# gyatskov/radix-sort

Hardware: AMD Instinct MI355X
Metric: Mkeys/s + scatter-pass HBM GB/s (% of peak), 2^28 uint32 keys (higher is better)
Workload: dtype u32; 1 GPU; 2^28 uint32 Random, 4-bit digits, 8 passes; keys_per_gpu=268435456, total_keys=268435456, parallelism=single GPU, verified=bit-exact vs RadixSortCPU (reference), all 268435456 keys

## Files before the change

radix-sort_amd/csrc/rsx_capi.hip:

```cpp
#include "radixsort_hip.h"
#ifdef RSX_EXPERIMENTS
#include "radixsort_hip_experiments.h"
#endif
#include "rsx_kernels.hpp"
#include "rsx_segmented.hpp"
#include "rsx_topk.hpp"
#include "rsx_select.hpp"
#include "rsx_unique.hpp"
#include "rsx_reduce.hpp"
#include "rsx_scan_by_key.hpp"

#include <hip/hip_runtime.h>

#include <algorithm>
#include <cstdio>
#include <cstdlib>
#include <cstring>
#include <limits>
#include <new>
#include <map>
#include <string>
#include <vector>

namespace {

thread_local std::string g_last_error;

int fail(int status, const char* what, hipError_t err = hipSuccess)
{
    g_last_error = what;
    if (err != hipSuccess) {
        g_last_error += ": ";
        g_last_error += hipGetErrorString(err);
    }
    std::fprintf(stderr, "[radixsort_hip] %s\n", g_last_error.c_str());
    return status;
}

#define RSX_TRY(expr, status)                                     \
    do {                                                          \
        const hipError_t rsx_err_ = (expr);                       \
        if (rsx_err_ != hipSuccess) {                             \
            return fail((status), #expr, rsx_err_);               \
        }                                                         \
    } while (0)

#ifndef RSX_TILE_THREADS
#define RSX_TILE_THREADS 256
#endif
#ifndef RSX_KPT
#define RSX_KPT 16
#endif
constexpr int kTileThreads = RSX_TILE_THREADS;
constexpr int kKeysPerThread = RSX_KPT;
constexpr int kTileKeys = kTileThreads * kKeysPerThread;
constexpr int kSmallKeysPerThread = 4;
#define RSX_PRODUCT_SHAPE (RSX_TILE_THREADS == 256 && RSX_KPT == 16)

enum Phase : int { PH_HISTO = 0, PH_SCAN = 1, PH_PASTE = 2, PH_REORDER = 3, PH_TOTAL = 4, PH_COUNT = 5 };

struct EventPair {
    int phase;
    hipEvent_t start, stop;
};

void stat_reset(rsx_phase_stat& s)
{
    s.min_ms = std::numeric_limits<double>::infinity();
    s.max_ms = -std::numeric_limits<double>::infinity();
    s.avg_ms = 0.0;
    s.sum_ms = 0.0;
    s.n = 0;
}

void stat_update(rsx_phase_stat& s, double ms)
{
    s.n += 1;
    s.sum_ms += ms;
    s.avg_ms = s.sum_ms / static_cast<double>(s.n);
    s.max_ms = std::max(s.max_ms, ms);
    s.min_ms = std::min(s.min_ms, ms);
}

}

struct GraphEntry {
    const void* in;
    const uint32_t* pin;
    uint64_t n;
    int cur, first, last, flags;
    uint64_t options_epoch;
    hipStream_t stream;
    hipGraphExec_t exec;
    int end_cur;
    const void* end_last_in;
    int end_last_shift;
};

struct rsx_engine {
    int device = 0;
    int key_bytes = 4;
    bool is_signed = false;
    int key_kind = RSX_KEY_UNSIGNED;
    bool descending = false;
    int codec_first = 0, codec_last = 0;
    bool has_payload = false;
    uint64_t capacity = 0;
    uint64_t n = 0;

    void* keys[2] = {nullptr, nullptr};
    uint32_t* perm[2] = {nullptr, nullptr};
    int cur = 0;
    void* result_keys = nullptr;
    uint32_t* result_perm = nullptr;

    uint32_t* table = nullptr;
    uint32_t* globsum = nullptr;
    uint32_t* globsum2 = nullptr;
    uint32_t* globsum_live = nullptr;
    int paste_scan = 1;
    int fused_scan = 1;
    unsigned long long* gsums = nullptr;
    uint32_t* scan_timeout = nullptr;
    uint32_t* scan_timeout_host = nullptr;
    uint32_t fused_scan_resident = 0;
    uint32_t fused_scan_limit = 0;
    bool table_valid = false;
    bool globsum_valid = false;
    uint32_t scan_epoch = 0;
    uint32_t* temp = nullptr;
    uint32_t* counts_next = nullptr;
#ifdef RSX_EXPERIMENTS
    uint32_t* counts_next2 = nullptr;
    uint32_t* scan_ready = nullptr;
    int inline_scan = 0;
    uint32_t inline_scan_max_groups = 64;
    uint32_t inline_scan_limit = 0;
#endif
#ifdef RSX_STAMPS
    unsigned long long* stamps = nullptr;
    int stamp_pass = -1;
#endif
    uint32_t* ref_table = nullptr;
    uint32_t* ref_globsum = nullptr;
    const void* counted_keys = nullptr;
    uint64_t counted_n = 0;
    int counted_shift = 0, counted_bits = 0;
    const void* last_in = nullptr;
    int last_shift = 0;
    int ref_diag = 0;
    uint64_t splitters[rsx::kMaxSplitters] = {};
    uint32_t nsplit = 0;
    bool result_external = false;
    void* final_keys_out = nullptr;
    uint32_t* final_perm_out = nullptr;
    unsigned long long* range_dev = nullptr;
    unsigned long long* range_host = nullptr;
    uint32_t* starts_dev = nullptr;
    uint32_t* starts_host = nullptr;
    uint64_t table_cap = 0;
#ifdef RSX_EXPERIMENTS
    struct BigBuf {
        void* base = nullptr;
        size_t size = 0;
        std::vector<hipMemGenericAllocationHandle_t> chunks;
    };
    std::vector<BigBuf> big;
    int alloc_mode = 0;
    size_t alloc_chunk = 0;
#endif
    rsx::MsdPlan* msd_plan = nullptr;
    rsx::MsdPlan* msd_plan_host = nullptr;
    uint32_t* msd_starts = nullptr;
    hipEvent_t msd_event = nullptr;
    hipEvent_t msd_scatter_event = nullptr;
    bool msd_scattered = false;
    hipEvent_t marks[RSX_MAX_MARKS] = {};
    std::map<int, hipEvent_t> order_events;
    const void* msd_keys = nullptr;
    uint64_t msd_n = 0;
    int msd_bits = 0, msd_world = 0;
    bool msd_planned = false;

    rsx::SegHeader* seg_hdr = nullptr;
    uint32_t* seg_temp = nullptr;
    uint32_t* seg_status_host = nullptr;
    uint32_t* seg_status = nullptr;
    uint64_t* seg_bsum = nullptr;
    uint32_t* seg_list = nullptr;
    rsx::SegLarge* seg_large = nullptr;
    uint32_t* seg_tstart = nullptr;
    uint32_t* seg_table = nullptr;
    uint32_t* seg_gsum = nullptr;
    uint32_t* seg_gsum2 = nullptr;
    uint64_t seg_bsum_cap = 0, seg_list_cap = 0, seg_large_cap = 0, seg_tstart_cap = 0, seg_table_cap = 0, seg_gsum_cap = 0, seg_gsum2_cap = 0;
    rsx::TopkState* topk_state = nullptr;
    uint32_t* topk_start = nullptr;
    uint32_t* topk_cont = nullptr;
    uint64_t topk_state_cap = 0, topk_start_cap = 0, topk_cont_cap = 0;
    uint32_t* uniq_iota = nullptr;
    uint64_t uniq_iota_cap = 0;
    uint64_t* red_part = nullptr;
    uint64_t red_part_cap = 0;

    hipStream_t stream = nullptr;
    bool own_stream = false;

    struct Pipeline {
        bool ready = false;
        void* in[2] = {nullptr, nullptr};
        void* out[2] = {nullptr, nullptr};
        uint32_t* pin[2] = {nullptr, nullptr};
        uint32_t* pout[2] = {nullptr, nullptr};
        hipStream_t s_in = nullptr, s_out = nullptr;
        hipEvent_t in_ready[2] = {nullptr, nullptr}, sorted[2] = {nullptr, nullptr}, out_done[2] = {nullptr, nullptr};
        uint64_t submitted = 0;
    } pipe;

    int profile = 0;
    int xcd_remap = 1;
    uint64_t options_epoch = 0;
    int64_t xcd_phase = -1;
    int lookahead = 1;
    int small_scan = 1;
    uint64_t radix8_min_keys = 1u << 19;
    int radix_bits = 4;
#ifdef RSX_EXPERIMENTS
    int reorder8_version = 1;
    int r8_stay = -1;
    int lds_atomics_ordered = -1;
    uint32_t* tickets8 = nullptr;
#endif
    long r8_extra_lds = -1;
    long reorder_extra_lds = -1;
    int reorder_wide = -1;
    int r8_wide = -1;
    int num_cus = 0;
    int r8_packed = 1;
    bool radix8_ready = false;
    uint32_t* counts8 = nullptr;
    uint32_t* table8 = nullptr;
    uint32_t* gsum8 = nullptr;
    uint32_t* csum8 = nullptr;
    uint32_t* cbase8 = nullptr;
    int self_scan = 1;
    uint32_t self_scan_max = 1024;
    uint32_t* cnt3[3] = {nullptr, nullptr, nullptr};
    uint64_t small_tile_max_keys = 1u << 19;
    int tile_sort = 1;
    int first_pass = 0;
    int last_pass = 0;

    int use_graph = 0;
    std::vector<GraphEntry> graphs;
    std::vector<EventPair> pending;
    std::vector<hipEvent_t> pool;
    rsx_phase_stat stats[PH_COUNT];

    uint32_t passes() const { return static_cast<uint32_t>(key_bytes * 8 / RSX_RADIX_BITS); }
    bool codec() const { return key_kind == RSX_KEY_FLOAT || descending; }
    uint64_t ntiles(uint64_t count) const { return (count + kTileKeys - 1) / kTileKeys; }
};

namespace {

struct Bracket {
    rsx_engine* e;
    int phase;
    hipEvent_t start = nullptr, stop = nullptr;
    bool on = false;
    Bracket(rsx_engine* eng, int ph) : e(eng), phase(ph)
    {
        if (e->profile == 0 || (e->profile == 2 && ph != PH_REORDER && ph != PH_TOTAL)) return;
        auto take = [&]() -> hipEvent_t {
            if (!e->pool.empty()) {
                hipEvent_t ev = e->pool.back();
                e->pool.pop_back();
                return ev;
            }
            hipEvent_t ev = nullptr;
            if (hipEventCreate(&ev) != hipSuccess) return nullptr;
            return ev;
        };
        start = take();
        stop = take();
        on = start && stop;
        if (on) (void)hipEventRecord(start, e->stream);
    }
    ~Bracket()
    {
        if (!on) return;
        (void)hipEventRecord(stop, e->stream);
        e->pending.push_back({phase, start, stop});
    }
};

int drain_events(rsx_engine* e)
{
    RSX_TRY(hipStreamSynchronize(e->stream), RSX_CALCULATION_FAILED);
    for (const EventPair& p : e->pending) {
        float ms = 0.f;
        if (hipEventElapsedTime(&ms, p.start, p.stop) == hipSuccess) {
            stat_update(e->stats[p.phase], static_cast<double>(ms));
        }
        e->pool.push_back(p.start);
        e->pool.push_back(p.stop);
    }
    e->pending.clear();
    return RSX_OK;
}

template <typename Key>
Key flip_mask(const rsx_engine* e)
{
    return (e->is_signed && !e->codec()) ? static_cast<Key>(Key{1} << (sizeof(Key) * 8 - 1)) : Key{0};
}

template <typename Key>
void order_consts(const rsx_engine* e, Key* a, Key* m)
{
    constexpr Key sign = static_cast<Key>(Key{1} << (sizeof(Key) * 8 - 1));
    if (e->key_kind == RSX_KEY_FLOAT) {
        *m = static_cast<Key>(~sign);
        *a = e->descending ? static_cast<Key>(~sign) : sign;
    } else {
        *m = Key{0};
        const Key flip = e->is_signed ? sign : Key{0};
        *a = e->descending ? static_cast<Key>(~flip) : flip;
    }
}

template <typename Key>
Key codec_decode_host(Key y, Key a, Key m)
{
    const Key z = y ^ a;
    const Key fill = (z >> (sizeof(Key) * 8 - 1)) ? static_cast<Key>(~Key{0}) : Key{0};
    return z ^ (fill & m);
}

constexpr int kEncode = 1, kDecode = 2;

template <typename Key>
rsx::KeyCodec<Key> key_codec(const rsx_engine* e, int cx)
{
    Key a = 0, m = 0;
    order_consts<Key>(e, &a, &m);
    rsx::KeyCodec<Key> c{};
    if (cx & kEncode) {
        c.ea = a;
        c.em = m;
    }
    if (cx & kDecode) {
        c.da = a;
        c.dm = m;
    }
    return c;
}

int pass_codec(const rsx_engine* e, int pass, int width, int first, int last)
{
    if (!e->codec()) return 0;
    return (pass == first ? kEncode : 0) | (pass + width == last ? kDecode : 0);
}
int pass_codec(const rsx_engine* e, int pass, int width)
{
    return pass_codec(e, pass, width, e->codec_first, e->codec_last);
}

int refuse_codec(const char* what)
{
    return fail(RSX_CALCULATION_FAILED, (std::string(what) + ": not available for float keys or descending order (the sharded sort and the partition passes take integer keys in ascending order)").c_str());
}

struct Grid {
    uint32_t ntiles, tiles_per_xcd, blocks;
    int remap;
};

Grid grid_for(const rsx_engine* e, uint64_t count, uint32_t tile_keys = kTileKeys)
{
    Grid g;
    g.ntiles = static_cast<uint32_t>((count + tile_keys - 1) / tile_keys);
    g.tiles_per_xcd = (g.ntiles + rsx::kNumXcd - 1) / rsx::kNumXcd;
    g.blocks = e->xcd_remap ? g.tiles_per_xcd * rsx::kNumXcd : g.ntiles;
    const uint64_t want = e->xcd_phase < 0 ? g.tiles_per_xcd / rsx::kNumXcd : static_cast<uint64_t>(e->xcd_phase);
    const uint32_t phase = (e->xcd_remap && (rsx::kNumXcd - 1) * want < g.tiles_per_xcd) ? static_cast<uint32_t>(want) : 0u;
    g.remap = (e->xcd_remap ? 1 : 0) | static_cast<int>(phase << 8);
    return g;
}

template <typename Key>
rsx::SplitSet<Key> split_set(const rsx_engine* e, uint32_t nsplit)
{
    rsx::SplitSet<Key> set{};
    for (uint32_t k = 0; k < nsplit && k < static_cast<uint32_t>(rsx::kMaxSplitters); ++k) set.s[k] = static_cast<Key>(e->splitters[k]);
    set.n = nsplit;
    return set;
}

template <typename Key, bool RANGED = false>
int launch_histogram(rsx_engine* e, const void* in, uint64_t count, int shift, uint32_t mask, Key lo = Key{0}, Key mul = Key{0}, uint32_t nsplit = 0,
                     int cx = 0)
{
    if (count == 0) return RSX_OK;
    e->counted_keys = nullptr;
    e->table_valid = true;
    e->globsum_valid = false;
    const Grid g = grid_for(e, count);
    Bracket b(e, PH_HISTO);
    if (!RANGED && (cx & kEncode)) {
        hipLaunchKernelGGL((rsx::histogram_kernel<Key, kTileThreads, kKeysPerThread, false, true>), dim3(g.blocks), dim3(kTileThreads), 0, e->stream,
                           static_cast<const Key*>(in), e->table, count, g.ntiles, g.tiles_per_xcd, g.remap, shift,
                           flip_mask<Key>(e), mask, lo, mul, split_set<Key>(e, nsplit), nullptr, nullptr, nullptr, key_codec<Key>(e, kEncode));
    } else {
        hipLaunchKernelGGL((rsx::histogram_kernel<Key, kTileThreads, kKeysPerThread, RANGED>), dim3(g.blocks), dim3(kTileThreads), 0, e->stream,
                           static_cast<const Key*>(in), e->table, count, g.ntiles, g.tiles_per_xcd, g.remap, shift,
                           flip_mask<Key>(e), mask, lo, mul, split_set<Key>(e, nsplit));
    }
    RSX_TRY(hipGetLastError(), RSX_CALCULATION_FAILED);
    return RSX_OK;
}

int launch_scan(rsx_engine* e, uint64_t count, bool from_counts = false, bool scan_level2 = true)
{
    if (count == 0) return RSX_OK;
    e->counted_keys = nullptr;
    const uint32_t ntiles = static_cast<uint32_t>(e->ntiles(count));
    const uint32_t ngroups = (ntiles + rsx::kScanTiles - 1) / rsx::kScanTiles;
    e->globsum_live = e->globsum;
    e->table_valid = true;
    e->globsum_valid = true;
    {
        Bracket b(e, PH_SCAN);
        if (from_counts) {
            hipLaunchKernelGGL((rsx::scan_blocks_kernel<true, true>), dim3(ngroups), dim3(rsx::kScanTiles), 0, e->stream, e->table, e->globsum,
                               ntiles, ngroups, e->counts_next);
        } else {
            hipLaunchKernelGGL((rsx::scan_blocks_kernel<false, false>), dim3(ngroups), dim3(rsx::kScanTiles), 0, e->stream, e->table, e->globsum,
                               ntiles, ngroups, static_cast<uint32_t*>(nullptr));
        }
    }
    RSX_TRY(hipGetLastError(), RSX_CALCULATION_FAILED);
    if (scan_level2) {
        Bracket b(e, PH_SCAN);
        hipLaunchKernelGGL(rsx::scan_globsum_kernel, dim3(1), dim3(rsx::kGlobsumThreads), 0, e->stream, e->globsum, e->temp,
                           static_cast<uint32_t>(RSX_RADIX) * ngroups);
    }
    RSX_TRY(hipGetLastError(), RSX_CALCULATION_FAILED);
    return RSX_OK;
}

int launch_paste_scan(rsx_engine* e, uint64_t count)
{
    if (count == 0) return RSX_OK;
    const uint32_t ntiles = static_cast<uint32_t>(e->ntiles(count));
    const uint32_t ngroups = (ntiles + rsx::kScanTiles - 1) / rsx::kScanTiles;
    e->globsum_live = e->globsum2;
    e->globsum_valid = true;
    Bracket b(e, PH_PASTE);
    hipLaunchKernelGGL(rsx::paste_scan_kernel, dim3(ngroups), dim3(rsx::kScanTiles), 0, e->stream, e->table, e->globsum, e->globsum2, e->temp,
                       ntiles, ngroups);
    RSX_TRY(hipGetLastError(), RSX_CALCULATION_FAILED);
    return RSX_OK;
}

bool launch_scan_fused(rsx_engine* e, uint64_t count, bool from_counts, int* rc)
{
    const uint32_t ntiles = static_cast<uint32_t>(e->ntiles(count));
    const uint32_t ngroups = (ntiles + rsx::kScanTiles - 1) / rsx::kScanTiles;
    if (!e->fused_scan || e->use_graph || count == 0 || ngroups > e->fused_scan_limit) return false;
    e->counted_keys = nullptr;
    e->globsum_live = e->globsum2;
    e->table_valid = true;
    e->globsum_valid = true;
    if (++e->scan_epoch == 0) e->scan_epoch = 1;
    {
        Bracket b(e, PH_SCAN);
        if (from_counts) {
            hipLaunchKernelGGL((rsx::scan_fused_kernel<true, true>), dim3(ngroups), dim3(rsx::kScanTiles), 0, e->stream, e->table, e->gsums, e->globsum2, e->temp,
                               ntiles, ngroups, e->counts_next, e->scan_epoch, e->scan_timeout);
        } else {
            hipLaunchKernelGGL((rsx::scan_fused_kernel<false, false>), dim3(ngroups), dim3(rsx::kScanTiles), 0, e->stream, e->table, e->gsums, e->globsum2, e->temp,
                               ntiles, ngroups, e->counts_next, e->scan_epoch, e->scan_timeout);
        }
    }
    *rc = hipGetLastError() == hipSuccess ? RSX_OK : fail(RSX_CALCULATION_FAILED, "scan_fused_kernel launch");
    return true;
}

bool launch_scan_small(rsx_engine* e, uint64_t count, bool from_counts, int* rc)
{
    const uint32_t ntiles = static_cast<uint32_t>(e->ntiles(count));
    if (!e->small_scan || count == 0 || ntiles > static_cast<uint32_t>(rsx::kSmallScanMaxTiles)) return false;
    e->counted_keys = nullptr;
    e->table_valid = true;
    e->globsum_valid = false;
    {
        Bracket b(e, PH_SCAN);
        if (from_counts) {
            hipLaunchKernelGGL((rsx::scan_small_kernel<true, true>), dim3(1), dim3(rsx::kSmallScanThreads), 0, e->stream, e->table, e->counts_next, e->temp, ntiles);
        } else {
            hipLaunchKernelGGL((rsx::scan_small_kernel<false, false>), dim3(1), dim3(rsx::kSmallScanThreads), 0, e->stream, e->table, e->counts_next, e->temp, ntiles);
        }
    }
    *rc = hipGetLastError() == hipSuccess ? RSX_OK : fail(RSX_CALCULATION_FAILED, "scan_small_kernel launch");
    return true;
}

int launch_paste(rsx_engine* e, uint64_t count)
{
    if (count == 0) return RSX_OK;
    const uint32_t ntiles = static_cast<uint32_t>(e->ntiles(count));
    const uint32_t ngroups = (ntiles + rsx::kScanTiles - 1) / rsx::kScanTiles;
    Bracket b(e, PH_PASTE);
    hipLaunchKernelGGL(rsx::paste_kernel, dim3(ngroups), dim3(rsx::kScanTiles), 0, e->stream, e->table, e->globsum, ntiles, ngroups);
    RSX_TRY(hipGetLastError(), RSX_CALCULATION_FAILED);
    return RSX_OK;
}

template <typename Key, bool PAYLOAD, bool LOOKAHEAD, bool RANGED = false, int KPT = kKeysPerThread, int THREADS = kTileThreads>
int launch_reorder_t(rsx_engine* e, const void* in, void* out, const uint32_t* pin, uint32_t* pout, uint64_t count, int shift,
                     uint32_t mask, int next_shift, Key lo = Key{0}, Key mul = Key{0}, uint32_t nsplit = 0,
                     rsx::SelfScanArgs self = rsx::SelfScanArgs{nullptr, nullptr, nullptr}, uint32_t* next_counts = nullptr, int cx = 0)
{
    using L = rsx::ReorderLayout<Key, THREADS, KPT>;
    const Grid g = grid_for(e, count, THREADS * KPT);
    e->last_in = in;
    e->last_shift = shift;
    Bracket b(e, PH_REORDER);
    const size_t lds = L::BYTES + (KPT != kKeysPerThread ? 0u : e->reorder_extra_lds >= 0 ? static_cast<size_t>(e->reorder_extra_lds) : (PAYLOAD && sizeof(Key) == 4 && !RANGED) ? (16u << 10) : 0u);
    if constexpr (!RANGED) {
        if (cx) {
            hipLaunchKernelGGL((rsx::reorder_kernel<Key, THREADS, KPT, PAYLOAD, LOOKAHEAD, false, false, true>), dim3(g.blocks), dim3(THREADS), lds,
                               e->stream, static_cast<const Key*>(in), static_cast<Key*>(out), pin, pout, e->table, count,
                               g.ntiles, g.tiles_per_xcd, g.remap, shift, flip_mask<Key>(e), mask,
                               next_counts ? next_counts : e->counts_next, next_shift, static_cast<const uint32_t*>(nullptr),
                               lo, mul, split_set<Key>(e, nsplit), self, rsx::InlineScanArgs{}, key_codec<Key>(e, cx));
            RSX_TRY(hipGetLastError(), RSX_CALCULATION_FAILED);
            return RSX_OK;
        }
    }
    hipLaunchKernelGGL((rsx::reorder_kernel<Key, THREADS, KPT, PAYLOAD, LOOKAHEAD, RANGED>), dim3(g.blocks), dim3(THREADS),
                       lds,
                       e->stream, static_cast<const Key*>(in), static_cast<Key*>(out), pin, pout, e->table, count,
                       g.ntiles, g.tiles_per_xcd, g.remap, shift, flip_mask<Key>(e), mask,
                       next_counts ? next_counts : e->counts_next, next_shift,
#ifdef RSX_STAMPS
                       (shift == e->stamp_pass * RSX_RADIX_BITS) ? reinterpret_cast<const uint32_t*>(e->stamps) : static_cast<const uint32_t*>(nullptr),
#else
                       static_cast<const uint32_t*>(nullptr),
#endif
                       lo, mul, split_set<Key>(e, nsplit), self);
    RSX_TRY(hipGetLastError(), RSX_CALCULATION_FAILED);
    return RSX_OK;
}

template <typename Key>
int launch_reorder(rsx_engine* e, const void* in, void* out, const uint32_t* pin, uint32_t* pout, uint64_t count, int shift,
                   uint32_t mask, int next_shift = -1, int cx = 0)
{
    const rsx::SelfScanArgs none{nullptr, nullptr, nullptr};
    if (count == 0) return RSX_OK;
    const bool payload = pin && pout;
#if RSX_PRODUCT_SHAPE
    if constexpr (sizeof(Key) == 8) {
        if (payload && (e->reorder_wide >= 0 ? e->reorder_wide != 0 : true)) {
            return next_shift >= 0 ? launch_reorder_t<Key, true, true, false, 8, 512>(e, in, out, pin, pout, count, shift, mask, next_shift, Key{0}, Key{0}, 0, none, nullptr, cx)
                                   : launch_reorder_t<Key, true, false, false, 8, 512>(e, in, out, pin, pout, count, shift, mask, 0, Key{0}, Key{0}, 0, none, nullptr, cx);
        }
    }
#endif
    if (next_shift >= 0) {
        return payload ? launch_reorder_t<Key, true, true>(e, in, out, pin, pout, count, shift, mask, next_shift, Key{0}, Key{0}, 0, none, nullptr, cx)
                       : launch_reorder_t<Key, false, true>(e, in, out, nullptr, nullptr, count, shift, mask, next_shift, Key{0}, Key{0}, 0, none, nullptr, cx);
    }
    return payload ? launch_reorder_t<Key, true, false>(e, in, out, pin, pout, count, shift, mask, 0, Key{0}, Key{0}, 0, none, nullptr, cx)
                   : launch_reorder_t<Key, false, false>(e, in, out, nullptr, nullptr, count, shift, mask, 0, Key{0}, Key{0}, 0, none, nullptr, cx);
}

int no_static_lds(const void* fn, const char* name)
{
    hipFuncAttributes attr;
    RSX_TRY(hipFuncGetAttributes(&attr, fn), RSX_KERNEL_CREATION_FAILED);
    if (attr.sharedSizeBytes != 0) return fail(RSX_KERNEL_CREATION_FAILED, (std::string(name) + ": static LDS in front of the dynamic array (the kernels address LDS from 0)").c_str());
    return RSX_OK;
}

int lds_base_probe(rsx_engine* e)
{
    uint32_t at = 1;
    RSX_TRY(hipMemsetAsync(e->temp + 4, 0xFF, 4, e->stream), RSX_KERNEL_CREATION_FAILED);
    hipLaunchKernelGGL(rsx::lds_base_probe_kernel, dim3(1), dim3(64), 256, e->stream, e->temp + 4);
    RSX_TRY(hipGetLastError(), RSX_KERNEL_CREATION_FAILED);
    RSX_TRY(hipMemcpyAsync(&at, e->temp + 4, 4, hipMemcpyDeviceToHost, e->stream), RSX_KERNEL_CREATION_FAILED);
    RSX_TRY(hipStreamSynchronize(e->stream), RSX_KERNEL_CREATION_FAILED);
    if (at != 0) return fail(RSX_KERNEL_CREATION_FAILED, "a kernel's dynamic LDS does not start at address 0 on this device");
    return RSX_OK;
}

template <typename Key, bool PAYLOAD, bool LOOKAHEAD, bool RANGED = false, int KPT = kKeysPerThread, int THREADS = kTileThreads, bool CODEC = false>
int allow_lds()
{
    using L = rsx::ReorderLayout<Key, THREADS, KPT>;
    const void* fn = reinterpret_cast<const void*>(&rsx::reorder_kernel<Key, THREADS, KPT, PAYLOAD, LOOKAHEAD, RANGED, false, CODEC>);
    RSX_TRY(hipFuncSetAttribute(fn, hipFuncAttributeMaxDynamicSharedMemorySize, static_cast<int>(L::BYTES) + (64 << 10)), RSX_INITIALIZATION_FAILED);
    return no_static_lds(fn, "reorder_kernel");
}

template <typename Key>
int run_pass(rsx_engine* e, const void* in, void* out, const uint32_t* pin, uint32_t* pout, uint64_t count, int shift, uint32_t mask, int cx = 0)
{
    int rc;
    if ((rc = launch_histogram<Key>(e, in, count, shift, mask, Key{0}, Key{0}, 0, cx)) != RSX_OK) return rc;
    if ((rc = launch_scan(e, count)) != RSX_OK) return rc;
    if ((rc = launch_paste(e, count)) != RSX_OK) return rc;
    return launch_reorder<Key>(e, in, out, pin, pout, count, shift, mask, -1, cx);
}

template <typename Key>
int run_ranged_pass(rsx_engine* e, const void* in, void* out, const uint32_t* pin, uint32_t* pout, uint64_t count, uint64_t lo, int shift,
                    uint64_t mul)
{
    const Key klo = static_cast<Key>(lo), kmul = static_cast<Key>(mul);
    int rc;
    if ((rc = launch_histogram<Key, true>(e, in, count, shift, RSX_RADIX - 1, klo, kmul)) != RSX_OK) return rc;
    if ((rc = launch_scan(e, count)) != RSX_OK) return rc;
    if ((rc = launch_paste(e, count)) != RSX_OK) return rc;
    if (pin && pout) return launch_reorder_t<Key, true, false, true>(e, in, out, pin, pout, count, shift, RSX_RADIX - 1, 0, klo, kmul);
    return launch_reorder_t<Key, false, false, true>(e, in, out, nullptr, nullptr, count, shift, RSX_RADIX - 1, 0, klo, kmul);
}

constexpr int kRangeBlocks = 2048;

template <typename Key>
int key_range(rsx_engine* e, const void* d_keys, uint64_t n, uint64_t* lo, uint64_t* hi)
{
    const uint32_t blocks = static_cast<uint32_t>(std::min<uint64_t>(kRangeBlocks, (n + 4095) / 4096));
    hipLaunchKernelGGL(rsx::key_range_kernel<Key>, dim3(blocks), dim3(rsx::kRangeThreads), 0, e->stream, static_cast<const Key*>(d_keys), n,
                       flip_mask<Key>(e), e->range_dev);
    RSX_TRY(hipGetLastError(), RSX_CALCULATION_FAILED);
    RSX_TRY(hipMemcpyAsync(e->range_host, e->range_dev, static_cast<size_t>(blocks) * 16, hipMemcpyDeviceToHost, e->stream), RSX_CALCULATION_FAILED);
    RSX_TRY(hipStreamSynchronize(e->stream), RSX_CALCULATION_FAILED);
    unsigned long long l = ~0ull, h = 0ull;
    for (uint32_t b = 0; b < blocks; ++b) {
        l = std::min(l, e->range_host[2 * b]);
        h = std::max(h, e->range_host[2 * b + 1]);
    }
    *lo = l;
    *hi = h;
    return RSX_OK;
}

template <typename Key, bool PAYLOAD>
int launch_tile_sort_t(rsx_engine* e, const void* in, void* out, void* before_last, const uint32_t* pin, uint32_t* pout, uint32_t* pbefore_last, uint64_t count)
{
    using L = rsx::TileSortLayout<Key, kTileThreads, kKeysPerThread>;
    Bracket b(e, PH_REORDER);
    if (e->codec()) {
        hipLaunchKernelGGL((rsx::tile_sort_kernel<Key, kTileThreads, kKeysPerThread, PAYLOAD, true>), dim3(1), dim3(kTileThreads), L::BYTES, e->stream,
                           static_cast<const Key*>(in), static_cast<Key*>(out), static_cast<Key*>(before_last), pin, pout, pbefore_last,
                           static_cast<uint32_t>(count), e->first_pass, e->last_pass, flip_mask<Key>(e), e->table, e->globsum, e->temp,
                           key_codec<Key>(e, pass_codec(e, e->first_pass, e->last_pass - e->first_pass)));
    } else {
        hipLaunchKernelGGL((rsx::tile_sort_kernel<Key, kTileThreads, kKeysPerThread, PAYLOAD>), dim3(1), dim3(kTileThreads), L::BYTES, e->stream,
                           static_cast<const Key*>(in), static_cast<Key*>(out), static_cast<Key*>(before_last), pin, pout, pbefore_last,
                           static_cast<uint32_t>(count), e->first_pass, e->last_pass, flip_mask<Key>(e), e->table, e->globsum, e->temp);
    }
    RSX_TRY(hipGetLastError(), RSX_CALCULATION_FAILED);
    return RSX_OK;
}

template <typename Key>
int sort_tile_enqueue(rsx_engine* e, const void* ext_keys, const uint32_t* ext_perm, uint64_t count)
{
    const int npasses = e->last_pass - e->first_pass;
    const void* in = ext_keys ? ext_keys : e->keys[e->cur];
    const uint32_t* pin = e->has_payload ? (ext_keys ? ext_perm : e->perm[e->cur]) : nullptr;
    const int first_dst = ext_keys ? e->cur : (e->cur ^ 1);
    const int final_buf = first_dst ^ ((npasses - 1) & 1);
    void* out = e->final_keys_out ? e->final_keys_out : e->keys[final_buf];
    uint32_t* pout = e->has_payload ? (e->final_keys_out ? e->final_perm_out : e->perm[final_buf]) : nullptr;
    void* before_last = npasses > 1 ? e->keys[final_buf ^ 1] : nullptr;
    uint32_t* pbefore_last = (npasses > 1 && e->has_payload) ? e->perm[final_buf ^ 1] : nullptr;
    Bracket whole(e, PH_TOTAL);
    e->counted_keys = nullptr;
    e->globsum_live = e->globsum;
    const int rc = e->has_payload ? launch_tile_sort_t<Key, true>(e, in, out, before_last, pin, pout, pbefore_last, count)
                                  : launch_tile_sort_t<Key, false>(e, in, out, before_last, nullptr, nullptr, nullptr, count);
    if (rc != RSX_OK) return rc;
    e->last_in = npasses > 1 ? before_last : in;
    e->last_shift = (e->last_pass - 1) * RSX_RADIX_BITS;
    e->table_valid = true;
    e->globsum_valid = true;
    e->result_external = e->final_keys_out != nullptr;
    if (e->final_keys_out) {
        e->result_keys = e->final_keys_out;
        e->result_perm = e->has_payload ? e->final_perm_out : nullptr;
    } else {
        e->cur = final_buf;
        e->result_keys = e->keys[e->cur];
        e->result_perm = e->has_payload ? e->perm[e->cur] : nullptr;
    }
    return RSX_OK;
}

template <typename Key, int KPT = kKeysPerThread>
int sort_selfscan_enqueue(rsx_engine* e, const void* ext_keys, const uint32_t* ext_perm, uint64_t count)
{
    const Grid g = grid_for(e, count, kTileThreads * KPT);
    const void* in = ext_keys ? ext_keys : e->keys[e->cur];
    const uint32_t* pin = e->has_payload ? (ext_keys ? ext_perm : e->perm[e->cur]) : nullptr;
    int dst = ext_keys ? e->cur : (e->cur ^ 1);
    Bracket whole(e, PH_TOTAL);
    e->counted_keys = nullptr;
    {
        Bracket b(e, PH_HISTO);
        if (pass_codec(e, e->first_pass, 1) & kEncode) {
            hipLaunchKernelGGL((rsx::histogram_kernel<Key, kTileThreads, KPT, false, true>), dim3(g.blocks), dim3(kTileThreads), 0, e->stream,
                               static_cast<const Key*>(in), e->table, count, g.ntiles, g.tiles_per_xcd, g.remap, e->first_pass * RSX_RADIX_BITS,
                               flip_mask<Key>(e), static_cast<uint32_t>(RSX_RADIX - 1), Key{0}, Key{0}, split_set<Key>(e, 0), e->cnt3[0], e->cnt3[1], e->cnt3[2],
                               key_codec<Key>(e, kEncode));
        } else {
            hipLaunchKernelGGL((rsx::histogram_kernel<Key, kTileThreads, KPT, false>), dim3(g.blocks), dim3(kTileThreads), 0, e->stream,
                               static_cast<const Key*>(in), e->table, count, g.ntiles, g.tiles_per_xcd, g.remap, e->first_pass * RSX_RADIX_BITS,
                               flip_mask<Key>(e), static_cast<uint32_t>(RSX_RADIX - 1), Key{0}, Key{0}, split_set<Key>(e, 0), e->cnt3[0], e->cnt3[1], e->cnt3[2]);
        }
        RSX_TRY(hipGetLastError(), RSX_CALCULATION_FAILED);
    }
    int i = 0;
    for (int pass = e->first_pass; pass < e->last_pass; ++pass, ++i) {
        const bool last = pass + 1 == e->last_pass;
        const bool to_caller = e->final_keys_out && last;
        void* out = to_caller ? e->final_keys_out : e->keys[dst];
        uint32_t* pout = e->has_payload ? (to_caller ? e->final_perm_out : e->perm[dst]) : nullptr;
        const int shift = pass * RSX_RADIX_BITS;
        const rsx::SelfScanArgs self{e->cnt3[i % 3], e->cnt3[(i + 2) % 3], (last && KPT == kKeysPerThread) ? e->table : nullptr};
        uint32_t* next = e->cnt3[(i + 1) % 3];
        const int cx = pass_codec(e, pass, 1);
        int rc;
        if (e->has_payload) {
            rc = last ? launch_reorder_t<Key, true, false, false, KPT>(e, in, out, pin, pout, count, shift, RSX_RADIX - 1, 0, Key{0}, Key{0}, 0, self, next, cx)
                      : launch_reorder_t<Key, true, true, false, KPT>(e, in, out, pin, pout, count, shift, RSX_RADIX - 1, shift + RSX_RADIX_BITS, Key{0}, Key{0}, 0, self, next, cx);
        } else {
            rc = last ? launch_reorder_t<Key, false, false, false, KPT>(e, in, out, nullptr, nullptr, count, shift, RSX_RADIX - 1, 0, Key{0}, Key{0}, 0, self, next, cx)
                      : launch_reorder_t<Key, false, true, false, KPT>(e, in, out, nullptr, nullptr, count, shift, RSX_RADIX - 1, shift + RSX_RADIX_BITS, Key{0}, Key{0}, 0, self, next, cx);
        }
        if (rc != RSX_OK) return rc;
        in = out;
        pin = pout;
        dst ^= 1;
    }
    e->table_valid = (KPT == kKeysPerThread);
    e->globsum_valid = false;
    if (in == e->keys[0] || in == e->keys[1]) e->cur = (in == e->keys[0]) ? 0 : 1;
    e->result_external = e->final_keys_out != nullptr;
    if (e->final_keys_out) {
        e->result_keys = e->final_keys_out;
        e->result_perm = e->has_payload ? e->final_perm_out : nullptr;
    } else {
        e->result_keys = e->keys[e->cur];
        e->result_perm = e->has_payload ? e->perm[e->cur] : nullptr;
    }
    return RSX_OK;
}

#if RSX_TILE_THREADS == 256
size_t r8_extra_lds_for(const rsx_engine* e, bool elem64, bool separate_payload)
{
    if (e->r8_extra_lds >= 0) return static_cast<size_t>(e->r8_extra_lds);
    if (!elem64) return separate_payload ? 0 : (4u << 10);
    if (separate_payload) return 16u << 10;
    return 8u << 10;
}

bool r8_wide_for(const rsx_engine* e, bool key64, bool has_payload)
{
    if (e->r8_wide >= 0) return e->r8_wide != 0;
    return key64 && !has_payload;
}

template <typename K, int THREADS, int KPT, bool PAYLOAD, bool PACKED32 = false, bool CODEC = false>
int allow_lds8(int extra)
{
    using L = rsx::Reorder8Layout<K, THREADS, KPT, PAYLOAD>;
    const void* fn = reinterpret_cast<const void*>(&rsx::reorder8_kernel<K, THREADS, KPT, PAYLOAD, PACKED32, CODEC>);
    RSX_TRY(hipFuncSetAttribute(fn, hipFuncAttributeMaxDynamicSharedMemorySize, static_cast<int>(L::BYTES) + extra), RSX_INITIALIZATION_FAILED);
    return no_static_lds(fn, "reorder8_kernel");
}

#ifdef RSX_EXPERIMENTS
template <typename Key> int ensure_radix8_experiments(rsx_engine* e, int extra);
template <typename Key> bool launch_reorder8_experiment(rsx_engine* e, const void* in, void* out, const uint32_t* pin, uint32_t* pout, uint64_t count, const Grid& g,
                                                        uint32_t chunk_groups, int shift, int byte_pass, bool first_of_chain, int* rc);
#endif

template <typename Key>
int ensure_radix8(rsx_engine* e)
{
    if (e->radix8_ready) return RSX_OK;
    const int extra = e->r8_extra_lds >= 0 ? static_cast<int>(e->r8_extra_lds) : (16 << 10);
    const size_t rows = static_cast<size_t>(e->ntiles(e->capacity)) * rsx::kRadix8 * 4;
    const size_t groups = ((e->ntiles(e->capacity) + rsx::kScan8Tiles - 1) / rsx::kScan8Tiles) * rsx::kRadix8 * 4;
    if (!e->counts8) RSX_TRY(hipMalloc(reinterpret_cast<void**>(&e->counts8), rows), RSX_INITIALIZATION_FAILED);
    if (!e->table8) RSX_TRY(hipMalloc(reinterpret_cast<void**>(&e->table8), rows), RSX_INITIALIZATION_FAILED);
    if (!e->gsum8) RSX_TRY(hipMalloc(reinterpret_cast<void**>(&e->gsum8), groups), RSX_INITIALIZATION_FAILED);
    if (!e->csum8) RSX_TRY(hipMalloc(reinterpret_cast<void**>(&e->csum8), rsx::kScan8MaxChunks * rsx::kRadix8 * 4), RSX_INITIALIZATION_FAILED);
    if (!e->cbase8) RSX_TRY(hipMalloc(reinterpret_cast<void**>(&e->cbase8), rsx::kScan8MaxChunks * rsx::kRadix8 * 4), RSX_INITIALIZATION_FAILED);
    int rc = allow_lds8<Key, kTileThreads, kKeysPerThread, false>(extra);
    if (rc == RSX_OK) rc = allow_lds8<Key, kTileThreads, kKeysPerThread, true>(extra);
    if (rc == RSX_OK) rc = allow_lds8<Key, 512, 8, false>(extra);
    if (rc == RSX_OK) rc = allow_lds8<Key, 512, 8, true>(extra);
    if constexpr (sizeof(Key) == 4) {
        if (rc == RSX_OK) rc = allow_lds8<uint64_t, kTileThreads, kKeysPerThread, false, true>(extra);
        if (rc == RSX_OK) rc = allow_lds8<uint64_t, 512, 8, false, true>(extra);
    }
    if (e->codec()) {
        if (rc == RSX_OK) rc = allow_lds8<Key, kTileThreads, kKeysPerThread, false, false, true>(extra);
        if (rc == RSX_OK) rc = allow_lds8<Key, kTileThreads, kKeysPerThread, true, false, true>(extra);
        if (rc == RSX_OK) rc = allow_lds8<Key, 512, 8, false, false, true>(extra);
        if (rc == RSX_OK) rc = allow_lds8<Key, 512, 8, true, false, true>(extra);
        if constexpr (sizeof(Key) == 4) {
            if (rc == RSX_OK) rc = allow_lds8<uint64_t, kTileThreads, kKeysPerThread, false, true, true>(extra);
            if (rc == RSX_OK) rc = allow_lds8<uint64_t, 512, 8, false, true, true>(extra);
        }
    }
#ifdef RSX_EXPERIMENTS
    if (rc == RSX_OK) rc = ensure_radix8_experiments<Key>(e, extra);
#endif
    if (rc != RSX_OK) return rc;
    e->radix8_ready = true;
    return RSX_OK;
}

template <typename K, int THREADS, int KPT, bool PAYLOAD, bool PACKED32 = false>
void launch_reorder8_v(rsx_engine* e, const dim3& grid, size_t lds, const void* in, void* out, const uint32_t* pin, uint32_t* pout, uint64_t count,
                       const Grid& g, uint32_t chunk_groups, int shift, K flip, int cx)
{
    using CK = typename std::conditional<PACKED32, uint32_t, K>::type;
    if (cx) {
        hipLaunchKernelGGL((rsx::reorder8_kernel<K, THREADS, KPT, PAYLOAD, PACKED32, true>), grid, dim3(THREADS), lds, e->stream,
                           static_cast<const K*>(in), static_cast<K*>(out), pin, pout, e->table8, e->gsum8, e->cbase8, chunk_groups,
                           count, g.ntiles, g.tiles_per_xcd, g.remap, shift, flip, key_codec<CK>(e, cx));
    } else {
        hipLaunchKernelGGL((rsx::reorder8_kernel<K, THREADS, KPT, PAYLOAD, PACKED32>), grid, dim3(THREADS), lds, e->stream,
                           static_cast<const K*>(in), static_cast<K*>(out), pin, pout, e->table8, e->gsum8, e->cbase8, chunk_groups,
                           count, g.ntiles, g.tiles_per_xcd, g.remap, shift, flip);
    }
}

template <typename Key>
int launch_reorder8(rsx_engine* e, const void* in, void* out, const uint32_t* pin, uint32_t* pout, uint64_t count, const Grid& g, uint32_t chunk_groups, int shift,
                    int cx = 0)
{
    const Key flip = flip_mask<Key>(e);
    e->last_in = nullptr;
    const bool packed = sizeof(Key) == 4 && e->has_payload && e->r8_packed;
    const bool wide = r8_wide_for(e, sizeof(Key) == 8, e->has_payload);
    const size_t wide_extra = e->r8_extra_lds >= 0 ? static_cast<size_t>(e->r8_extra_lds) : 0;
    const dim3 grid(g.blocks);
    constexpr size_t lds_packed = rsx::Reorder8Layout<uint64_t, kTileThreads, kKeysPerThread>::BYTES, lds_packed_wide = rsx::Reorder8Layout<uint64_t, 512, 8, false>::BYTES;
    constexpr size_t lds_pay = rsx::Reorder8Layout<Key, kTileThreads, kKeysPerThread, true>::BYTES, lds_pay_wide = rsx::Reorder8Layout<Key, 512, 8, true>::BYTES;
    constexpr size_t lds_keys = rsx::Reorder8Layout<Key, kTileThreads, kKeysPerThread>::BYTES, lds_keys_wide = rsx::Reorder8Layout<Key, 512, 8, false>::BYTES;
    if (packed) {
        if (wide) {
            launch_reorder8_v<uint64_t, 512, 8, false, true>(e, grid, lds_packed_wide + wide_extra, in, out, pin, pout, count, g, chunk_groups, shift,
                                                             static_cast<uint64_t>(flip), cx);
        } else {
            launch_reorder8_v<uint64_t, kTileThreads, kKeysPerThread, false, true>(e, grid, lds_packed + r8_extra_lds_for(e, true, false), in, out, pin, pout, count, g,
                                                                                   chunk_groups, shift, static_cast<uint64_t>(flip), cx);
        }
    } else if (e->has_payload) {
        if (wide) {
            launch_reorder8_v<Key, 512, 8, true>(e, grid, lds_pay_wide + wide_extra, in, out, pin, pout, count, g, chunk_groups, shift, flip, cx);
        } else {
            launch_reorder8_v<Key, kTileThreads, kKeysPerThread, true>(e, grid, lds_pay + r8_extra_lds_for(e, sizeof(Key) == 8, true), in, out, pin, pout, count, g,
                                                                      chunk_groups, shift, flip, cx);
        }
    } else {
        if (wide) {
            launch_reorder8_v<Key, 512, 8, false>(e, grid, lds_keys_wide + wide_extra, in, out, nullptr, nullptr, count, g, chunk_groups, shift, flip, cx);
        } else {
            launch_reorder8_v<Key, kTileThreads, kKeysPerThread, false>(e, grid, lds_keys + r8_extra_lds_for(e, sizeof(Key) == 8, false), in, out, nullptr, nullptr,
                                                                       count, g, chunk_groups, shift, flip, cx);
        }
    }
    RSX_TRY(hipGetLastError(), RSX_CALCULATION_FAILED);
    return RSX_OK;
}

struct Scan8Shape {
    uint32_t ngroups, chunk_groups, nchunks;
};
Scan8Shape scan8_shape(uint32_t ntiles)
{
    Scan8Shape s;
    s.ngroups = (ntiles + rsx::kScan8Tiles - 1) / rsx::kScan8Tiles;
    s.chunk_groups = std::max<uint32_t>(64u, (s.ngroups + rsx::kScan8MaxChunks - 1) / rsx::kScan8MaxChunks);
    s.nchunks = (s.ngroups + s.chunk_groups - 1) / s.chunk_groups;
    return s;
}

template <typename Key>
int launch_count8(rsx_engine* e, const void* in, uint64_t count, const Grid& g, const Scan8Shape& s, int shift, int cx = 0)
{
    e->msd_keys = nullptr;
    {
        Bracket b(e, PH_HISTO);
        if (cx & kEncode) {
            hipLaunchKernelGGL((rsx::histogram8_kernel<Key, kTileThreads, kKeysPerThread, true>), dim3(g.blocks), dim3(kTileThreads), 0, e->stream,
                               static_cast<const Key*>(in), e->counts8, count, g.ntiles, g.tiles_per_xcd, g.remap, shift, flip_mask<Key>(e), key_codec<Key>(e, kEncode));
        } else {
            hipLaunchKernelGGL((rsx::histogram8_kernel<Key, kTileThreads, kKeysPerThread>), dim3(g.blocks), dim3(kTileThreads), 0, e->stream,
                               static_cast<const Key*>(in), e->counts8, count, g.ntiles, g.tiles_per_xcd, g.remap, shift, flip_mask<Key>(e));
        }
    }
    {
        Bracket b(e, PH_SCAN);
        hipLaunchKernelGGL(rsx::scan8_blocks_kernel, dim3(s.ngroups), dim3(rsx::kRadix8), 0, e->stream, e->counts8, e->table8, e->gsum8, g.ntiles);
    }
    {
        Bracket b(e, PH_SCAN);
        if (s.nchunks == 1) {
            hipLaunchKernelGGL(rsx::scan8_chunks_kernel<true>, dim3(1), dim3(rsx::kRadix8), 0, e->stream, e->gsum8, e->csum8, s.ngroups, s.chunk_groups, e->cbase8, e->temp);
        } else {
            hipLaunchKernelGGL(rsx::scan8_chunks_kernel<false>, dim3(s.nchunks), dim3(rsx::kRadix8), 0, e->stream, e->gsum8, e->csum8, s.ngroups, s.chunk_groups, e->cbase8, e->temp);
            hipLaunchKernelGGL(rsx::scan8_top_kernel, dim3(1), dim3(rsx::kRadix8), 0, e->stream, e->csum8, e->cbase8, e->temp, s.nchunks);
        }
    }
    RSX_TRY(hipGetLastError(), RSX_CALCULATION_FAILED);
    return RSX_OK;
}

template <typename Key>
int sort8_chain_enqueue(rsx_engine* e, const void* ext_keys, const uint32_t* ext_perm, uint64_t count)
{
    const Grid g = grid_for(e, count);
    const Scan8Shape s = scan8_shape(g.ntiles);
    if (!e->radix8_ready) return fail(RSX_INITIALIZATION_FAILED, "sort8_chain_enqueue: the 8-bit tables were not allocated (ensure_radix8)");
    const void* in = ext_keys ? ext_keys : e->keys[e->cur];
    const uint32_t* pin = e->has_payload ? (ext_keys ? ext_perm : e->perm[e->cur]) : nullptr;
    int dst = ext_keys ? e->cur : (e->cur ^ 1);
    Bracket whole(e, PH_TOTAL);
    e->counted_keys = nullptr;
    for (int pass = e->first_pass; pass < e->last_pass; pass += 2) {
        const bool to_caller = e->final_keys_out && pass + 2 == e->last_pass;
        void* out = to_caller ? e->final_keys_out : e->keys[dst];
        uint32_t* pout = e->has_payload ? (to_caller ? e->final_perm_out : e->perm[dst]) : nullptr;
        const int shift = pass * RSX_RADIX_BITS;
        const int cx = pass_codec(e, pass, 2);
        int rc = launch_count8<Key>(e, in, count, g, s, shift, cx);
        if (rc != RSX_OK) return rc;
        {
            Bracket b(e, PH_REORDER);
#ifdef RSX_EXPERIMENTS
            if (e->codec() || !launch_reorder8_experiment<Key>(e, in, out, pin, pout, count, g, s.chunk_groups, shift, pass / 2, pass == e->first_pass, &rc))
#endif
                rc = launch_reorder8<Key>(e, in, out, pin, pout, count, g, s.chunk_groups, shift, cx);
        }
        if (rc != RSX_OK) return rc;
        in = out;
        pin = pout;
        dst ^= 1;
    }
    e->table_valid = false;
    e->globsum_valid = false;
    if (in == e->keys[0] || in == e->keys[1]) e->cur = (in == e->keys[0]) ? 0 : 1;
    e->result_external = e->final_keys_out != nullptr;
    if (e->final_keys_out) {
        e->result_keys = e->final_keys_out;
        e->result_perm = e->has_payload ? e->final_perm_out : nullptr;
    } else {
        e->result_keys = e->keys[e->cur];
        e->result_perm = e->has_payload ? e->perm[e->cur] : nullptr;
    }
    return RSX_OK;
}

#endif

#ifdef RSX_EXPERIMENTS
template <typename Key> int sort_inline_enqueue(rsx_engine* e, const void* ext_keys, const uint32_t* ext_perm, uint64_t count);
bool inline_scan_takes(const rsx_engine* e, uint64_t count);
#endif

template <typename Key>
int sort_chain_passes(rsx_engine* e, const void* ext_keys, const uint32_t* ext_perm, uint64_t count);

template <typename Key>
int sort_chain_enqueue(rsx_engine* e, const void* ext_keys, const uint32_t* ext_perm, uint64_t count)
{
    e->codec_first = e->first_pass;
    e->codec_last = e->last_pass;
    return sort_chain_passes<Key>(e, ext_keys, ext_perm, count);
}

template <typename Key>
int sort_chain_passes(rsx_engine* e, const void* ext_keys, const uint32_t* ext_perm, uint64_t count)
{
#if RSX_TILE_THREADS == 256
    if (e->radix_bits == 8 && count > e->radix8_min_keys && e->first_pass < e->last_pass && (e->first_pass & 1) == 0 && (e->last_pass & 1) == 0) {
        return sort8_chain_enqueue<Key>(e, ext_keys, ext_perm, count);
    }
    if (e->radix_bits == 8 && count > e->radix8_min_keys && (e->first_pass & 1) == 0 && (e->last_pass & 1) == 1 && e->last_pass - e->first_pass >= 3) {
        const int first = e->first_pass, last = e->last_pass;
        void* const keys_out = e->final_keys_out;
        uint32_t* const perm_out = e->final_perm_out;
        e->last_pass = last - 1;
        e->final_keys_out = nullptr;
        e->final_perm_out = nullptr;
        int rc = sort8_chain_enqueue<Key>(e, ext_keys, ext_perm, count);
        e->last_pass = last;
        e->final_keys_out = keys_out;
        e->final_perm_out = perm_out;
        if (rc != RSX_OK) return rc;
        e->first_pass = last - 1;
        rc = sort_chain_passes<Key>(e, nullptr, nullptr, count);
        e->first_pass = first;
        return rc;
    }
#endif
#if RSX_PRODUCT_SHAPE
    if (e->tile_sort && e->profile != 1 && count > 0 && count <= static_cast<uint64_t>(kTileKeys) && e->first_pass < e->last_pass) {
        return sort_tile_enqueue<Key>(e, ext_keys, ext_perm, count);
    }
#endif
    if (e->self_scan && e->lookahead && count > static_cast<uint64_t>(kTileKeys) && e->ntiles(count) <= e->self_scan_max && e->first_pass < e->last_pass) {
        if (count <= e->small_tile_max_keys) return sort_selfscan_enqueue<Key, kSmallKeysPerThread>(e, ext_keys, ext_perm, count);
        return sort_selfscan_enqueue<Key>(e, ext_keys, ext_perm, count);
    }
#if defined(RSX_EXPERIMENTS) && RSX_PRODUCT_SHAPE
    if (!e->codec() && inline_scan_takes(e, count)) return sort_inline_enqueue<Key>(e, ext_keys, ext_perm, count);
#endif
    const void* in = ext_keys ? ext_keys : e->keys[e->cur];
    const uint32_t* pin = e->has_payload ? (ext_keys ? ext_perm : e->perm[e->cur]) : nullptr;
    int dst = ext_keys ? e->cur : (e->cur ^ 1);
    Bracket whole(e, PH_TOTAL);
    if (e->lookahead && count > 0) {
        RSX_TRY(hipMemsetAsync(e->counts_next, 0, static_cast<size_t>(e->ntiles(count)) * RSX_RADIX * 4, e->stream), RSX_CALCULATION_FAILED);
    }
    for (int pass = e->first_pass; pass < e->last_pass; ++pass) {
        const bool to_caller = e->final_keys_out && pass + 1 == e->last_pass;
        void* out = to_caller ? e->final_keys_out : e->keys[dst];
        uint32_t* pout = e->has_payload ? (to_caller ? e->final_perm_out : e->perm[dst]) : nullptr;
        const int shift = pass * RSX_RADIX_BITS;
        const int cx = pass_codec(e, pass, 1);
        int rc;
        if (!e->lookahead) {
            rc = run_pass<Key>(e, in, out, pin, pout, count, shift, RSX_RADIX - 1, cx);
        } else {
            const bool first = pass == e->first_pass;
            rc = first ? launch_histogram<Key>(e, in, count, shift, RSX_RADIX - 1, Key{0}, Key{0}, 0, cx) : RSX_OK;
            bool pasted = false;
            if (rc == RSX_OK) pasted = launch_scan_small(e, count, !first, &rc);
            if (rc == RSX_OK && !pasted) pasted = launch_scan_fused(e, count, !first, &rc);
            const bool merged = e->paste_scan != 0;
            if (rc == RSX_OK && !pasted) rc = launch_scan(e, count, !first, !merged);
            const bool last = pass + 1 == e->last_pass;
            if (rc == RSX_OK && !pasted) rc = merged ? launch_paste_scan(e, count) : launch_paste(e, count);
            const int next_shift = last ? -1 : shift + RSX_RADIX_BITS;
            if (rc == RSX_OK) rc = launch_reorder<Key>(e, in, out, pin, pout, count, shift, RSX_RADIX - 1, next_shift, cx);
        }
        if (rc != RSX_OK) return rc;
        in = out;
        pin = pout;
        dst ^= 1;
    }
    if (in == e->keys[0] || in == e->keys[1]) {
        e->cur = (in == e->keys[0]) ? 0 : 1;
    }
    e->result_external = e->final_keys_out != nullptr;
    if (e->final_keys_out) {
        e->result_keys = e->final_keys_out;
        e->result_perm = e->has_payload ? e->final_perm_out : nullptr;
    } else {
        e->result_keys = e->keys[e->cur];
        e->result_perm = e->has_payload ? e->perm[e->cur] : nullptr;
    }
    return RSX_OK;
}

constexpr uint64_t kGraphMaxKeys = 1ull << 22;

template <typename Key>
int sort_chain(rsx_engine* e, const void* ext_keys, const uint32_t* ext_perm, uint64_t count)
{
#if RSX_TILE_THREADS == 256
    if (e->radix_bits == 8 && count > e->radix8_min_keys) {
        const int rc8 = ensure_radix8<Key>(e);
        if (rc8 != RSX_OK) return rc8;
    }
#endif
    const bool graphable = e->use_graph && e->profile == 0 && count > 0 && count <= kGraphMaxKeys && e->stream != nullptr && !e->final_keys_out;
    if (!graphable) return sort_chain_enqueue<Key>(e, ext_keys, ext_perm, count);
    GraphEntry key{};
    key.in = ext_keys;
    key.pin = ext_perm;
    key.n = count;
    key.cur = e->cur;
    key.first = e->first_pass;
    key.last = e->last_pass;
    key.flags = (e->lookahead ? 1 : 0) | (e->xcd_remap ? 2 : 0) | (e->small_scan ? 16 : 0);
    key.options_epoch = e->options_epoch;
    key.stream = e->stream;
    for (const GraphEntry& g : e->graphs) {
        if (g.in == key.in && g.pin == key.pin && g.n == key.n && g.cur == key.cur && g.first == key.first && g.last == key.last &&
            g.flags == key.flags && g.options_epoch == key.options_epoch && g.stream == key.stream) {
            RSX_TRY(hipGraphLaunch(g.exec, e->stream), RSX_CALCULATION_FAILED);
            e->cur = g.end_cur;
            e->last_in = g.end_last_in;
            e->last_shift = g.end_last_shift;
            e->result_external = false;
            e->result_keys = e->keys[e->cur];
            e->result_perm = e->has_payload ? e->perm[e->cur] : nullptr;
            return RSX_OK;
        }
    }
    hipGraph_t graph = nullptr;
    if (hipStreamBeginCapture(e->stream, hipStreamCaptureModeThreadLocal) != hipSuccess) {
        (void)hipGetLastError();
        e->use_graph = 0;
        return sort_chain_enqueue<Key>(e, ext_keys, ext_perm, count);
    }
    const int rc = sort_chain_enqueue<Key>(e, ext_keys, ext_perm, count);
    const hipError_t end = hipStreamEndCapture(e->stream, &graph);
    if (rc != RSX_OK || end != hipSuccess || !graph) {
        if (graph) (void)hipGraphDestroy(graph);
        return rc != RSX_OK ? rc : fail(RSX_CALCULATION_FAILED, "hipStreamEndCapture", end);
    }
    hipGraphExec_t exec = nullptr;
    const hipError_t inst = hipGraphInstantiate(&exec, graph, nullptr, nullptr, 0);
    (void)hipGraphDestroy(graph);
    if (inst != hipSuccess) return fail(RSX_CALCULATION_FAILED, "hipGraphInstantiate", inst);
    key.exec = exec;
    key.end_cur = e->cur;
    key.end_last_in = e->last_in;
    key.end_last_shift = e->last_shift;
    if (e->graphs.size() >= 8) {
        (void)hipGraphExecDestroy(e->graphs.front().exec);
        e->graphs.erase(e->graphs.begin());
    }
    e->graphs.push_back(key);
    RSX_TRY(hipGraphLaunch(exec, e->stream), RSX_CALCULATION_FAILED);
    return RSX_OK;
}

template <typename Key>
int sort_chain_keys_only(rsx_engine* e, const void* ext_keys, uint64_t count)
{
    const bool saved = e->has_payload;
    e->has_payload = false;
    const int rc = sort_chain<Key>(e, ext_keys, nullptr, count);
    e->has_payload = saved;
    return rc;
}

int check_scan_timeout(rsx_engine* e, int status)
{
    if (e->seg_status_host) {
        volatile uint32_t* bad = e->seg_status_host;
        const uint32_t v = *bad;
        if (v != 0) {
            *bad = 0;
            return fail(status, ("rsx_segmented_sort / rsx_segmented_topk / rsx_segmented_select: segment " + std::to_string(v - 1) + " has off[s+1] < off[s] or off[s+1] > n; it was neither read nor "
                                 "written (the first such segment of the call; reported once; the engine remains usable)").c_str());
        }
    }
    if (!e->scan_timeout_host) return RSX_OK;
    volatile uint32_t* flag = e->scan_timeout_host;
    if (*flag != 0) {
        *flag = 0;
        return fail(status, "the fused table scan timed out waiting for a group sum: the result of that sort is undefined (reported once; the engine remains usable)");
    }
    return RSX_OK;
}
bool aligned16(const void* p)
{
    return (reinterpret_cast<uintptr_t>(p) & 15u) == 0;
}

bool overlaps(const void* a, uint64_t abytes, const void* b, uint64_t bbytes)
{
    const uintptr_t a0 = reinterpret_cast<uintptr_t>(a), b0 = reinterpret_cast<uintptr_t>(b);
    return a && b && abytes && bbytes && a0 < b0 + bbytes && b0 < a0 + abytes;
}

int alias_of(const void* p, uint64_t bytes, void* const bufs[2], uint64_t buf_bytes, int* which)
{
    for (int i = 0; i < 2; ++i) {
        if (!bufs[i] || !overlaps(p, bytes, bufs[i], buf_bytes)) continue;
        if (p == bufs[i]) {
            *which = i;
            return 1;
        }
        return -1;
    }
    return 0;
}

int bind_device(const rsx_engine* e, int status)
{
    RSX_TRY(hipSetDevice(e->device), status);
    return RSX_OK;
}

#ifdef RSX_EXPERIMENTS
hipError_t big_alloc(rsx_engine* e, void** out, size_t bytes);
bool big_free(rsx_engine* e, void* p);
#else
hipError_t big_alloc(rsx_engine*, void** out, size_t bytes)
{
    *out = nullptr;
    return hipMalloc(out, bytes);
}

bool big_free(rsx_engine*, void* p)
{
    return !p || hipFree(p) == hipSuccess;
}
#endif

#ifdef RSX_EXPERIMENTS
#include "capi_experiments.inc"
#endif

struct EnvKnob {
    const char* name;
    const char* meaning;
    void (*apply)(rsx_engine* e, const char* value);
};
constexpr long kb_or_policy(const char* v, int max_kb)
{
    return std::atoi(v) < 0 ? -1L : static_cast<long>(std::min(max_kb, std::atoi(v))) * 1024;
}
const EnvKnob kEnvKnobs[] = {
    {"RSX_XCD_REMAP", "0: workgroup b takes tile b (default 1: XCD-contiguous tile ranges)", [](rsx_engine* e, const char* v) { e->xcd_remap = std::atoi(v) != 0; }},
    {"RSX_XCD_PHASE", "tiles by which consecutive XCDs enter their range staggered (-1: an eighth of a range)", [](rsx_engine* e, const char* v) { e->xcd_phase = std::atoll(v); }},
    {"RSX_LOOKAHEAD", "0: every pass runs histogram -> scan -> paste -> reorder (default 1: RSX_OPT_LOOKAHEAD)", [](rsx_engine* e, const char* v) { e->lookahead = std::atoi(v) != 0; }},
    {"RSX_GRAPH", "1: small sorts replay a captured hipGraph (RSX_OPT_GRAPH, default 0)", [](rsx_engine* e, const char* v) { e->use_graph = std::atoi(v) != 0; }},
    {"RSX_SMALL_SCAN", "0: no one-workgroup table scan (RSX_OPT_SMALL_SCAN)", [](rsx_engine* e, const char* v) { e->small_scan = std::atoi(v) != 0; }},
    {"RSX_TILE_SORT", "0: no one-launch sort of inputs up to one tile (RSX_OPT_TILE_SORT)", [](rsx_engine* e, const char* v) { e->tile_sort = std::atoi(v) != 0; }},
    {"RSX_SELF_SCAN", "0: small tables get scan launches (RSX_OPT_SELF_SCAN)", [](rsx_engine* e, const char* v) { e->self_scan = std::atoi(v) != 0; }},
    {"RSX_SELF_SCAN_MAX", "largest table, in tiles, of the self-scan chain (RSX_OPT_SELF_SCAN_MAX_TILES)",
     [](rsx_engine* e, const char* v) { e->self_scan_max = std::min<uint32_t>(static_cast<uint32_t>(std::atoi(v)), rsx::kSelfScanMaxTiles); }},
    {"RSX_SMALL_TILE_MAX_KEYS", "self-scan sorts up to this many keys use 1024-key tiles (RSX_OPT_SMALL_TILE_MAX_KEYS)",
     [](rsx_engine* e, const char* v) { e->small_tile_max_keys = std::min<uint64_t>(std::strtoull(v, nullptr, 10), static_cast<uint64_t>(rsx::kSelfScanMaxTiles) * kTileThreads * kSmallKeysPerThread); }},
    {"RSX_PASTE_SCAN", "0: scan #2 gets a launch of its own in the two-launch table scan", [](rsx_engine* e, const char* v) { e->paste_scan = std::atoi(v) != 0; }},
    {"RSX_FUSED_SCAN", "0: never the one-launch table scan (RSX_OPT_FUSED_SCAN)", [](rsx_engine* e, const char* v) { e->fused_scan = std::atoi(v) != 0; }},
    {"RSX_RADIX_BITS", "8: byte-wide passes in the sort chain (RSX_OPT_RADIX_BITS)", [](rsx_engine* e, const char* v) { e->radix_bits = std::atoi(v) == 8 ? 8 : 4; }},
    {"RSX_RADIX8_MIN_KEYS", "8-bit passes only above this many keys (default 2^19)", [](rsx_engine* e, const char* v) { e->radix8_min_keys = std::max<uint64_t>(std::strtoull(v, nullptr, 10), kTileKeys); }},
    {"RSX_REORDER_EXTRA_LDS_KB", "unused dynamic LDS per 4-bit scatter workgroup = fewer per CU (-1: per-variant policy)", [](rsx_engine* e, const char* v) { e->reorder_extra_lds = kb_or_policy(v, 64); }},
    {"RSX_REORDER_WIDE", "4-bit scatter of 64-bit keys + payload on 512 x 8 (0 / 1, -1: policy = on)", [](rsx_engine* e, const char* v) { e->reorder_wide = std::max(-1, std::min(1, std::atoi(v))); }},
    {"RSX_R8_EXTRA_LDS_KB", "the same for the 8-bit scatter (-1: per-variant policy)", [](rsx_engine* e, const char* v) { e->r8_extra_lds = kb_or_policy(v, 96); }},
    {"RSX_R8_PACKED", "0: uint32 key and payload travel apart through the 8-bit scatter (default 1: one 64-bit element)", [](rsx_engine* e, const char* v) { e->r8_packed = std::atoi(v) != 0; }},
    {"RSX_R8_WIDE", "8-bit scatter on 512 x 8 (0 / 1, -1: policy = 64-bit keys without payload)", [](rsx_engine* e, const char* v) { e->r8_wide = std::max(-1, std::min(1, std::atoi(v))); }},
#ifdef RSX_EXPERIMENTS
    {"RSX_ALLOC_MODE", "experiments: key buffers as VMM chunks mapped in creation (1) or shuffled (2) order", [](rsx_engine* e, const char* v) { e->alloc_mode = std::max(0, std::min(2, std::atoi(v))); }},
    {"RSX_ALLOC_CHUNK_MB", "experiments: chunk size of RSX_ALLOC_MODE", [](rsx_engine* e, const char* v) { e->alloc_chunk = static_cast<size_t>(std::max(0, std::atoi(v))) << 20; }},
#endif
};

void apply_environment(rsx_engine* e)
{
    for (const EnvKnob& k : kEnvKnobs) {
        if (const char* v = std::getenv(k.name)) k.apply(e, v);
    }
}

}

#define RSX_BY_KEY(e, call32, call64) ((e)->key_bytes == 4 ? (call32) : (call64))

extern "C" {

const char* rsx_last_error(void)
{
    return g_last_error.c_str();
}

const char* rsx_version(void)
{
    return "radixsort_hip 0.1 (gfx950; tile 256x16; 4-bit LSD)";
}

int rsx_device_count(int* count)
{
    if (!count) return fail(RSX_INITIALIZATION_FAILED, "rsx_device_count: null argument");
    *count = 0;
    int c = 0;
    const hipError_t err = hipGetDeviceCount(&c);
    if (err != hipSuccess) {
        return fail(RSX_INITIALIZATION_FAILED, "hipGetDeviceCount", err);
    }
    *count = c;
    return RSX_OK;
}

int rsx_device_name(int device, char* buf, size_t buflen)
{
    if (!buf || buflen == 0) return fail(RSX_INITIALIZATION_FAILED, "rsx_device_name: null buffer");
    hipDeviceProp_t prop;
    RSX_TRY(hipGetDeviceProperties(&prop, device), RSX_INITIALIZATION_FAILED);
    std::snprintf(buf, buflen, "%s (%s, %d CUs)", prop.name, prop.gcnArchName, prop.multiProcessorCount);
    return RSX_OK;
}

int rsx_create(rsx_engine** out, int device, int key_bytes, int key_kind, int has_payload, uint64_t capacity)
{
    if (!out) return fail(RSX_INITIALIZATION_FAILED, "rsx_create: null out pointer");
    *out = nullptr;
    if (key_bytes != 4 && key_bytes != 8) return fail(RSX_INITIALIZATION_FAILED, "rsx_create: key_bytes must be 4 or 8");
    if (key_kind < RSX_KEY_UNSIGNED || key_kind > RSX_KEY_FLOAT)
        return fail(RSX_INITIALIZATION_FAILED, "rsx_create: key_kind must be RSX_KEY_UNSIGNED (0), RSX_KEY_SIGNED (1) or RSX_KEY_FLOAT (2)");
    if (capacity == 0 || capacity > 0xFFFFFFFFull) {
        return fail(RSX_RESIZE_FAILED, "rsx_create: capacity must be in [1, 2^32-1] (32-bit slots)");
    }
    int count = 0;
    if (rsx_device_count(&count) != RSX_OK || count <= 0) {
        return fail(RSX_INITIALIZATION_FAILED, "rsx_create: no HIP device (this library has no CPU fallback)");
    }
    if (device < 0 || device >= count) return fail(RSX_INITIALIZATION_FAILED, "rsx_create: device ordinal out of range");

    rsx_engine* e = new (std::nothrow) rsx_engine();
    if (!e) return fail(RSX_HOST_BUFFERS_FAILED, "rsx_create: out of host memory");
    e->device = device;
    e->key_bytes = key_bytes;
    e->key_kind = key_kind;
    e->is_signed = key_kind == RSX_KEY_SIGNED;
    e->has_payload = has_payload != 0;
    e->capacity = capacity;
    e->n = 0;
    e->last_pass = static_cast<int>(e->passes());
    for (auto& s : e->stats) stat_reset(s);
    apply_environment(e);

    auto bail = [&](int status, const char* what, hipError_t err) {
        rsx_destroy(e);
        return fail(status, what, err);
    };
    hipError_t err;
    if ((err = hipSetDevice(device)) != hipSuccess) return bail(RSX_INITIALIZATION_FAILED, "hipSetDevice", err);
    if ((err = hipStreamCreateWithFlags(&e->stream, hipStreamNonBlocking)) != hipSuccess)
        return bail(RSX_INITIALIZATION_FAILED, "hipStreamCreate", err);
    e->own_stream = true;

    const size_t key_buf = static_cast<size_t>(capacity) * key_bytes;
    for (int i = 0; i < 2; ++i) {
        if ((err = big_alloc(e, &e->keys[i], key_buf)) != hipSuccess) return bail(RSX_INITIALIZATION_FAILED, "allocation of a key buffer", err);
        if (e->has_payload) {
            if ((err = big_alloc(e, reinterpret_cast<void**>(&e->perm[i]), static_cast<size_t>(capacity) * 4)) != hipSuccess)
                return bail(RSX_INITIALIZATION_FAILED, "hipMalloc(permutations)", err);
        }
    }
    e->table_cap = static_cast<uint64_t>(RSX_RADIX) * e->ntiles(capacity);
    if ((e->ntiles(capacity) + rsx::kScanTiles - 1) / rsx::kScanTiles > rsx::kMaxScanGroups) {
        return bail(RSX_RESIZE_FAILED, "rsx_create: capacity exceeds the two-level table scan", hipSuccess);
    }
    const size_t table_alloc = ((e->ntiles(capacity) + rsx::kScanTiles - 1) / rsx::kScanTiles) * rsx::kScanTiles * RSX_RADIX * 4;
    if ((err = hipMalloc(reinterpret_cast<void**>(&e->table), table_alloc)) != hipSuccess)
        return bail(RSX_INITIALIZATION_FAILED, "hipMalloc(histograms)", err);
    if ((err = hipMalloc(reinterpret_cast<void**>(&e->counts_next), table_alloc)) != hipSuccess)
        return bail(RSX_INITIALIZATION_FAILED, "hipMalloc(look-ahead counts)", err);
#ifdef RSX_EXPERIMENTS
    {
        const size_t second = std::min<size_t>(table_alloc, static_cast<size_t>(rsx::kFusedScanMaxGroups) * rsx::kScanTiles * RSX_RADIX * 4);
        if ((err = hipMalloc(reinterpret_cast<void**>(&e->counts_next2), second)) != hipSuccess)
            return bail(RSX_INITIALIZATION_FAILED, "hipMalloc(second look-ahead counts)", err);
        if ((err = hipMemsetAsync(e->counts_next2, 0, second, e->stream)) != hipSuccess)
            return bail(RSX_INITIALIZATION_FAILED, "hipMemsetAsync(second look-ahead counts)", err);
        if ((err = hipMalloc(reinterpret_cast<void**>(&e->scan_ready), rsx::kFusedScanMaxGroups * 4)) != hipSuccess)
            return bail(RSX_INITIALIZATION_FAILED, "hipMalloc(scan ready words)", err);
        if ((err = hipMemsetAsync(e->scan_ready, 0, rsx::kFusedScanMaxGroups * 4, e->stream)) != hipSuccess)
            return bail(RSX_INITIALIZATION_FAILED, "hipMemsetAsync(scan ready words)", err);
    }
#endif
#ifdef RSX_STAMPS
    if ((err = hipMalloc(reinterpret_cast<void**>(&e->stamps), e->ntiles(capacity) * 16 * 8)) != hipSuccess)
        return bail(RSX_INITIALIZATION_FAILED, "hipMalloc(stamps)", err);
    if (const char* env = std::getenv("RSX_STAMP_PASS")) e->stamp_pass = std::atoi(env);
#endif
    if ((err = hipMalloc(reinterpret_cast<void**>(&e->globsum), rsx::kMaxScanBlocks * 4)) != hipSuccess)
        return bail(RSX_INITIALIZATION_FAILED, "hipMalloc(globsum)", err);
    if ((err = hipMalloc(reinterpret_cast<void**>(&e->globsum2), rsx::kMaxScanBlocks * 4)) != hipSuccess)
        return bail(RSX_INITIALIZATION_FAILED, "hipMalloc(globsum2)", err);
    e->globsum_live = e->globsum;
    if ((err = hipMalloc(reinterpret_cast<void**>(&e->temp), 64)) != hipSuccess)
        return bail(RSX_INITIALIZATION_FAILED, "hipMalloc(temp)", err);
    for (int i = 0; i < 3; ++i) {
        if ((err = hipMalloc(reinterpret_cast<void**>(&e->cnt3[i]), rsx::kSelfScanMaxTiles * RSX_RADIX * 4)) != hipSuccess)
            return bail(RSX_INITIALIZATION_FAILED, "hipMalloc(self-scan counts)", err);
    }
    if ((err = hipMalloc(reinterpret_cast<void**>(&e->gsums), rsx::kFusedScanMaxGroups * RSX_RADIX * 8)) != hipSuccess)
        return bail(RSX_INITIALIZATION_FAILED, "hipMalloc(group sums)", err);
    if ((err = hipMemsetAsync(e->gsums, 0, rsx::kFusedScanMaxGroups * RSX_RADIX * 8, e->stream)) != hipSuccess)
        return bail(RSX_INITIALIZATION_FAILED, "hipMemsetAsync(group sums)", err);
    if ((err = hipHostMalloc(reinterpret_cast<void**>(&e->scan_timeout_host), 64, hipHostMallocMapped)) != hipSuccess)
        return bail(RSX_HOST_BUFFERS_FAILED, "hipHostMalloc(scan timeout flag)", err);
    e->scan_timeout_host[0] = 0;
    if ((err = hipHostGetDevicePointer(reinterpret_cast<void**>(&e->scan_timeout), e->scan_timeout_host, 0)) != hipSuccess)
        return bail(RSX_HOST_BUFFERS_FAILED, "hipHostGetDevicePointer(scan timeout flag)", err);
    {
        int per_cu = 0, cus = 0;
        if ((err = hipOccupancyMaxActiveBlocksPerMultiprocessor(&per_cu, reinterpret_cast<const void*>(&rsx::scan_fused_kernel<true, true>), rsx::kScanTiles, 0)) != hipSuccess)
            return bail(RSX_INITIALIZATION_FAILED, "hipOccupancyMaxActiveBlocksPerMultiprocessor(scan_fused_kernel)", err);
        if ((err = hipDeviceGetAttribute(&cus, hipDeviceAttributeMultiprocessorCount, device)) != hipSuccess)
            return bail(RSX_INITIALIZATION_FAILED, "hipDeviceGetAttribute(multiProcessorCount)", err);
        e->num_cus = cus;
        e->fused_scan_resident = static_cast<uint32_t>(std::max(per_cu, 0)) * static_cast<uint32_t>(std::max(cus, 0));
        e->fused_scan_limit = std::min<uint32_t>(e->fused_scan_resident / 2, rsx::kFusedScanMaxGroups);
        if (const char* env = std::getenv("RSX_FUSED_SCAN_MAX_GROUPS"))
            e->fused_scan_limit = std::min<uint32_t>(static_cast<uint32_t>(std::max(0, std::atoi(env))), std::min<uint32_t>(e->fused_scan_resident, rsx::kFusedScanMaxGroups));
    }
    if ((err = hipMalloc(reinterpret_cast<void**>(&e->ref_table), rsx::kRefTable * 4)) != hipSuccess)
        return bail(RSX_INITIALIZATION_FAILED, "hipMalloc(ref table)", err);
    if ((err = hipMalloc(reinterpret_cast<void**>(&e->ref_globsum), rsx::kRefSplit * 4)) != hipSuccess)
        return bail(RSX_INITIALIZATION_FAILED, "hipMalloc(ref globsum)", err);
    if ((err = hipMalloc(reinterpret_cast<void**>(&e->range_dev), kRangeBlocks * 16)) != hipSuccess)
        return bail(RSX_INITIALIZATION_FAILED, "hipMalloc(range)", err);
    if ((err = hipHostMalloc(reinterpret_cast<void**>(&e->range_host), kRangeBlocks * 16, hipHostMallocDefault)) != hipSuccess)
        return bail(RSX_HOST_BUFFERS_FAILED, "hipHostMalloc(range)", err);
    if ((err = hipMalloc(reinterpret_cast<void**>(&e->starts_dev), RSX_RADIX * 4)) != hipSuccess)
        return bail(RSX_INITIALIZATION_FAILED, "hipMalloc(starts)", err);
    if ((err = hipHostMalloc(reinterpret_cast<void**>(&e->starts_host), RSX_RADIX * 4, hipHostMallocDefault)) != hipSuccess)
        return bail(RSX_HOST_BUFFERS_FAILED, "hipHostMalloc(starts)", err);
    if ((err = hipMemsetAsync(e->globsum, 0, rsx::kMaxScanBlocks * 4, e->stream)) != hipSuccess)
        return bail(RSX_INITIALIZATION_FAILED, "hipMemsetAsync(globsum)", err);

    int rc = lds_base_probe(e);
#if RSX_PRODUCT_SHAPE
    if (rc == RSX_OK) {
        auto allow_tile = [](const void* fn, size_t bytes) { return hipFuncSetAttribute(fn, hipFuncAttributeMaxDynamicSharedMemorySize, static_cast<int>(bytes)); };
        using L32 = rsx::TileSortLayout<uint32_t, kTileThreads, kKeysPerThread>;
        using L64 = rsx::TileSortLayout<uint64_t, kTileThreads, kKeysPerThread>;
        if (allow_tile(reinterpret_cast<const void*>(&rsx::tile_sort_kernel<uint32_t, kTileThreads, kKeysPerThread, false>), L32::BYTES) != hipSuccess ||
            allow_tile(reinterpret_cast<const void*>(&rsx::tile_sort_kernel<uint32_t, kTileThreads, kKeysPerThread, true>), L32::BYTES) != hipSuccess ||
            allow_tile(reinterpret_cast<const void*>(&rsx::tile_sort_kernel<uint64_t, kTileThreads, kKeysPerThread, false>), L64::BYTES) != hipSuccess ||
            allow_tile(reinterpret_cast<const void*>(&rsx::tile_sort_kernel<uint64_t, kTileThreads, kKeysPerThread, true>), L64::BYTES) != hipSuccess ||
            allow_tile(reinterpret_cast<const void*>(&rsx::tile_sort_kernel<uint32_t, kTileThreads, kKeysPerThread, false, true>), L32::BYTES) != hipSuccess ||
            allow_tile(reinterpret_cast<const void*>(&rsx::tile_sort_kernel<uint32_t, kTileThreads, kKeysPerThread, true, true>), L32::BYTES) != hipSuccess ||
            allow_tile(reinterpret_cast<const void*>(&rsx::tile_sort_kernel<uint64_t, kTileThreads, kKeysPerThread, false, true>), L64::BYTES) != hipSuccess ||
            allow_tile(reinterpret_cast<const void*>(&rsx::tile_sort_kernel<uint64_t, kTileThreads, kKeysPerThread, true, true>), L64::BYTES) != hipSuccess)
            rc = fail(RSX_INITIALIZATION_FAILED, "hipFuncSetAttribute(tile_sort_kernel)");
    }
#endif
#if RSX_PRODUCT_SHAPE
    if (rc == RSX_OK) rc = allow_lds<uint64_t, true, false, false, 8, 512>();
    if (rc == RSX_OK) rc = allow_lds<uint64_t, true, true, false, 8, 512>();
    if (rc == RSX_OK) rc = allow_lds<uint64_t, true, false, false, 8, 512, true>();
    if (rc == RSX_OK) rc = allow_lds<uint64_t, true, true, false, 8, 512, true>();
#endif
    if (rc == RSX_OK) rc = allow_lds<uint32_t, false, false>();
    if (rc == RSX_OK) rc = allow_lds<uint32_t, true, false>();
    if (rc == RSX_OK) rc = allow_lds<uint64_t, false, false>();
    if (rc == RSX_OK) rc = allow_lds<uint64_t, true, false>();
    if (rc == RSX_OK) rc = allow_lds<uint32_t, false, true>();
    if (rc == RSX_OK) rc = allow_lds<uint32_t, true, true>();
    if (rc == RSX_OK) rc = allow_lds<uint64_t, false, true>();
    if (rc == RSX_OK) rc = allow_lds<uint64_t, true, true>();
    if (rc == RSX_OK) rc = allow_lds<uint32_t, false, false, true>();
    if (rc == RSX_OK) rc = allow_lds<uint32_t, true, false, true>();
    if (rc == RSX_OK) rc = allow_lds<uint64_t, false, false, true>();
    if (rc == RSX_OK) rc = allow_lds<uint64_t, true, false, true>();
    if (rc == RSX_OK) rc = allow_lds<uint32_t, false, false, false, kKeysPerThread, kTileThreads, true>();
    if (rc == RSX_OK) rc = allow_lds<uint32_t, true, false, false, kKeysPerThread, kTileThreads, true>();
    if (rc == RSX_OK) rc = allow_lds<uint64_t, false, false, false, kKeysPerThread, kTileThreads, true>();
    if (rc == RSX_OK) rc = allow_lds<uint64_t, true, false, false, kKeysPerThread, kTileThreads, true>();
    if (rc == RSX_OK) rc = allow_lds<uint32_t, false, true, false, kKeysPerThread, kTileThreads, true>();
    if (rc == RSX_OK) rc = allow_lds<uint32_t, true, true, false, kKeysPerThread, kTileThreads, true>();
    if (rc == RSX_OK) rc = allow_lds<uint64_t, false, true, false, kKeysPerThread, kTileThreads, true>();
    if (rc == RSX_OK) rc = allow_lds<uint64_t, true, true, false, kKeysPerThread, kTileThreads, true>();
    if (rc != RSX_OK) {
        rsx_destroy(e);
        return rc;
    }
    e->result_keys = e->keys[0];
    e->result_perm = e->perm[0];
    if (std::getenv("RSX_DEBUG_PTRS")) std::fprintf(stderr, "[radixsort_hip] keys[0]=%p keys[1]=%p table=%p counts_next=%p\n", e->keys[0], e->keys[1], static_cast<void*>(e->table), static_cast<void*>(e->counts_next));
    *out = e;
    return RSX_OK;
}

int rsx_destroy(rsx_engine* e)
{
    if (!e) return RSX_OK;
    int status = RSX_OK;
    if (hipSetDevice(e->device) != hipSuccess) status = RSX_CLEANUP_FAILED;
    if (e->stream) (void)hipStreamSynchronize(e->stream);
    for (const EventPair& p : e->pending) {
        (void)hipEventDestroy(p.start);
        (void)hipEventDestroy(p.stop);
    }
    for (hipEvent_t ev : e->pool) (void)hipEventDestroy(ev);
    for (const GraphEntry& g : e->graphs) (void)hipGraphExecDestroy(g.exec);
    for (int i = 0; i < 2; ++i) {
        if (!big_free(e, e->keys[i])) status = RSX_CLEANUP_FAILED;
        if (!big_free(e, e->perm[i])) status = RSX_CLEANUP_FAILED;
    }
    if (e->table && hipFree(e->table) != hipSuccess) status = RSX_CLEANUP_FAILED;
    if (e->counts_next && hipFree(e->counts_next) != hipSuccess) status = RSX_CLEANUP_FAILED;
#ifdef RSX_EXPERIMENTS
    if (e->counts_next2 && hipFree(e->counts_next2) != hipSuccess) status = RSX_CLEANUP_FAILED;
    if (e->scan_ready && hipFree(e->scan_ready) != hipSuccess) status = RSX_CLEANUP_FAILED;
    if (e->tickets8 && hipFree(e->tickets8) != hipSuccess) status = RSX_CLEANUP_FAILED;
#endif
    if (e->globsum && hipFree(e->globsum) != hipSuccess) status = RSX_CLEANUP_FAILED;
    if (e->globsum2 && hipFree(e->globsum2) != hipSuccess) status = RSX_CLEANUP_FAILED;
    if (e->temp && hipFree(e->temp) != hipSuccess) status = RSX_CLEANUP_FAILED;
    if (e->gsums && hipFree(e->gsums) != hipSuccess) status = RSX_CLEANUP_FAILED;
    for (int i = 0; i < 3; ++i) {
        if (e->cnt3[i] && hipFree(e->cnt3[i]) != hipSuccess) status = RSX_CLEANUP_FAILED;
    }
    if (e->counts8 && hipFree(e->counts8) != hipSuccess) status = RSX_CLEANUP_FAILED;
    if (e->table8 && hipFree(e->table8) != hipSuccess) status = RSX_CLEANUP_FAILED;
    if (e->gsum8 && hipFree(e->gsum8) != hipSuccess) status = RSX_CLEANUP_FAILED;
    if (e->csum8 && hipFree(e->csum8) != hipSuccess) status = RSX_CLEANUP_FAILED;
    if (e->cbase8 && hipFree(e->cbase8) != hipSuccess) status = RSX_CLEANUP_FAILED;
    if (e->scan_timeout_host && hipHostFree(e->scan_timeout_host) != hipSuccess) status = RSX_CLEANUP_FAILED;
    if (e->starts_dev && hipFree(e->starts_dev) != hipSuccess) status = RSX_CLEANUP_FAILED;
    if (e->msd_plan && hipFree(e->msd_plan) != hipSuccess) status = RSX_CLEANUP_FAILED;
    for (void* p : {static_cast<void*>(e->seg_hdr), static_cast<void*>(e->seg_temp), static_cast<void*>(e->seg_bsum), static_cast<void*>(e->seg_list),
                    static_cast<void*>(e->seg_large), static_cast<void*>(e->seg_tstart), static_cast<void*>(e->seg_table), static_cast<void*>(e->seg_gsum),
                    static_cast<void*>(e->seg_gsum2), static_cast<void*>(e->topk_state), static_cast<void*>(e->topk_start),
                    static_cast<void*>(e->topk_cont), static_cast<void*>(e->uniq_iota), static_cast<void*>(e->red_part)}) {
        if (p && hipFree(p) != hipSuccess) status = RSX_CLEANUP_FAILED;
    }
    if (e->seg_status_host && hipHostFree(e->seg_status_host) != hipSuccess) status = RSX_CLEANUP_FAILED;
    if (e->msd_starts && hipFree(e->msd_starts) != hipSuccess) status = RSX_CLEANUP_FAILED;
    if (e->msd_plan_host && hipHostFree(e->msd_plan_host) != hipSuccess) status = RSX_CLEANUP_FAILED;
    if (e->msd_event) (void)hipEventDestroy(e->msd_event);
    if (e->msd_scatter_event) (void)hipEventDestroy(e->msd_scatter_event);
    for (auto& kv : e->order_events) if (kv.second) (void)hipEventDestroy(kv.second);
    for (hipEvent_t ev : e->marks) if (ev) (void)hipEventDestroy(ev);
    if (e->range_dev && hipFree(e->range_dev) != hipSuccess) status = RSX_CLEANUP_FAILED;
    if (e->ref_table && hipFree(e->ref_table) != hipSuccess) status = RSX_CLEANUP_FAILED;
    if (e->ref_globsum && hipFree(e->ref_globsum) != hipSuccess) status = RSX_CLEANUP_FAILED;
    if (e->range_host && hipHostFree(e->range_host) != hipSuccess) status = RSX_CLEANUP_FAILED;
    if (e->starts_host && hipHostFree(e->starts_host) != hipSuccess) status = RSX_CLEANUP_FAILED;
    if (e->pipe.s_in) (void)hipStreamSynchronize(e->pipe.s_in);
    if (e->pipe.s_out) (void)hipStreamSynchronize(e->pipe.s_out);
    for (int i = 0; i < 2; ++i) {
        if (e->pipe.in[i] && hipFree(e->pipe.in[i]) != hipSuccess) status = RSX_CLEANUP_FAILED;
        if (e->pipe.out[i] && hipFree(e->pipe.out[i]) != hipSuccess) status = RSX_CLEANUP_FAILED;
        if (e->pipe.pin[i] && hipFree(e->pipe.pin[i]) != hipSuccess) status = RSX_CLEANUP_FAILED;
        if (e->pipe.pout[i] && hipFree(e->pipe.pout[i]) != hipSuccess) status = RSX_CLEANUP_FAILED;
        if (e->pipe.in_ready[i]) (void)hipEventDestroy(e->pipe.in_ready[i]);
        if (e->pipe.sorted[i]) (void)hipEventDestroy(e->pipe.sorted[i]);
        if (e->pipe.out_done[i]) (void)hipEventDestroy(e->pipe.out_done[i]);
    }
    if (e->pipe.s_in && hipStreamDestroy(e->pipe.s_in) != hipSuccess) status = RSX_CLEANUP_FAILED;
    if (e->pipe.s_out && hipStreamDestroy(e->pipe.s_out) != hipSuccess) status = RSX_CLEANUP_FAILED;
    if (e->own_stream && e->stream && hipStreamDestroy(e->stream) != hipSuccess) status = RSX_CLEANUP_FAILED;
    delete e;
    return status;
}

int rsx_set_stream(rsx_engine* e, void* hip_stream)
{
    if (!e) return fail(RSX_INITIALIZATION_FAILED, "rsx_set_stream: null engine");
    if (bind_device(e, RSX_INITIALIZATION_FAILED) != RSX_OK) return RSX_INITIALIZATION_FAILED;
    const int rc = drain_events(e);
    if (rc != RSX_OK) return rc;
    for (const GraphEntry& g : e->graphs) (void)hipGraphExecDestroy(g.exec);
    e->graphs.clear();
    if (e->own_stream && e->stream) {
        RSX_TRY(hipStreamDestroy(e->stream), RSX_INITIALIZATION_FAILED);
    }
    e->stream = static_cast<hipStream_t>(hip_stream);
    e->own_stream = false;
    return RSX_OK;
}

int rsx_get_stream(const rsx_engine* e, void** hip_stream)
{
    if (!e || !hip_stream) return fail(RSX_INITIALIZATION_FAILED, "rsx_get_stream: null argument");
    *hip_stream = static_cast<void*>(e->stream);
    return RSX_OK;
}

int rsx_set_option(rsx_engine* e, int option, int64_t value)
{
    if (!e) return fail(RSX_INITIALIZATION_FAILED, "rsx_set_option: null engine");
    ++e->options_epoch;
    switch (option) {
    case RSX_OPT_PROFILE: e->profile = value < 0 || value > 2 ? 1 : static_cast<int>(value); return RSX_OK;
    case RSX_OPT_XCD_REMAP: e->xcd_remap = value != 0; return RSX_OK;
    case RSX_OPT_LOOKAHEAD: e->lookahead = value != 0; return RSX_OK;
    case RSX_OPT_REF_DIAGNOSTICS:
        if (value != 0 && e->codec()) return refuse_codec("RSX_OPT_REF_DIAGNOSTICS");
        e->ref_diag = value != 0;
        return RSX_OK;
    case RSX_OPT_DESCENDING:
        if (value != 0 && e->ref_diag) return refuse_codec("RSX_OPT_DESCENDING with RSX_OPT_REF_DIAGNOSTICS");
        e->descending = value != 0;
        e->radix8_ready = false;
        return RSX_OK;
    case RSX_OPT_GRAPH: e->use_graph = value != 0; return RSX_OK;
    case RSX_OPT_SMALL_SCAN: e->small_scan = value != 0; return RSX_OK;
    case RSX_OPT_TILE_SORT: e->tile_sort = value != 0; return RSX_OK;
    case RSX_OPT_FUSED_SCAN: e->fused_scan = value != 0; return RSX_OK;
#ifdef RSX_EXPERIMENTS
    case RSX_XOPT_REORDER8_KERNEL:
        if (value < 1 || value > 3) return fail(RSX_CALCULATION_FAILED, "rsx_set_option: the 8-bit scatter kernel is 1, 2 or 3");
        e->reorder8_version = static_cast<int>(value);
        return RSX_OK;
    case RSX_XOPT_REORDER8_STAY:
        if (value < -1 || value > 8) return fail(RSX_CALCULATION_FAILED, "rsx_set_option: workgroups per CU of the staying 8-bit scatter: -1 / 0 (off) .. 8");
        e->r8_stay = static_cast<int>(value);
        return RSX_OK;
    case RSX_XOPT_INLINE_SCAN:
        e->inline_scan = value != 0;
        if (e->inline_scan && e->inline_scan_limit == 0) {
            if (bind_device(e, RSX_INITIALIZATION_FAILED) != RSX_OK) return RSX_INITIALIZATION_FAILED;
            return RSX_BY_KEY(e, inline_scan_prepare<uint32_t>(e), inline_scan_prepare<uint64_t>(e));
        }
        return RSX_OK;
    case RSX_XOPT_INLINE_SCAN_MAX_GROUPS:
        if (value < 0) return fail(RSX_CALCULATION_FAILED, "rsx_set_option: negative group count");
        e->inline_scan_max_groups = static_cast<uint32_t>(std::min<int64_t>(value, rsx::kFusedScanMaxGroups));
        return RSX_OK;
    case RSX_XOPT_DEBUG_RAISE_SCAN_TIMEOUT:
        if (bind_device(e, RSX_CALCULATION_FAILED) != RSX_OK) return RSX_CALCULATION_FAILED;
        hipLaunchKernelGGL(rsx::raise_flag_kernel, dim3(1), dim3(64), 0, e->stream, e->scan_timeout);
        RSX_TRY(hipGetLastError(), RSX_CALCULATION_FAILED);
        return RSX_OK;
#endif
    case RSX_OPT_FUSED_SCAN_MAX_GROUPS:
        if (value < -1) return fail(RSX_CALCULATION_FAILED, "rsx_set_option: negative group count");
        e->fused_scan_limit = value < 0 ? std::min<uint32_t>(e->fused_scan_resident / 2, rsx::kFusedScanMaxGroups)
                                        : static_cast<uint32_t>(std::min<int64_t>(value, std::min<uint32_t>(e->fused_scan_resident, rsx::kFusedScanMaxGroups)));
        return RSX_OK;
    case RSX_OPT_SELF_SCAN: e->self_scan = value != 0; return RSX_OK;
    case RSX_OPT_SMALL_TILE_MAX_KEYS:
        if (value < 0) return fail(RSX_CALCULATION_FAILED, "rsx_set_option: negative key count");
        e->small_tile_max_keys = std::min<uint64_t>(static_cast<uint64_t>(value), static_cast<uint64_t>(rsx::kSelfScanMaxTiles) * kTileThreads * kSmallKeysPerThread);
        return RSX_OK;
    case RSX_OPT_SELF_SCAN_MAX_TILES:
        if (value < 0) return fail(RSX_CALCULATION_FAILED, "rsx_set_option: negative tile count");
        e->self_scan_max = static_cast<uint32_t>(std::min<int64_t>(value, rsx::kSelfScanMaxTiles));
        return RSX_OK;
    case RSX_OPT_XCD_PHASE:
        if (value < -1 || value > (1 << 22)) return fail(RSX_CALCULATION_FAILED, "rsx_set_option: XCD phase out of range");
        e->xcd_phase = value;
        return RSX_OK;
    case RSX_OPT_RADIX_BITS:
        if (value != 4 && value != 8) return fail(RSX_CALCULATION_FAILED, "rsx_set_option: digit width must be 4 or 8 bits");
        e->radix_bits = static_cast<int>(value);
#if RSX_TILE_THREADS == 256
        if (value == 8 && e->capacity > e->radix8_min_keys) {
            if (bind_device(e, RSX_INITIALIZATION_FAILED) != RSX_OK) return RSX_INITIALIZATION_FAILED;
            return RSX_BY_KEY(e, ensure_radix8<uint32_t>(e), ensure_radix8<uint64_t>(e));
        }
#endif
        return RSX_OK;
    case RSX_OPT_FIRST_PASS:
        if (value < 0 || value > e->passes()) return fail(RSX_CALCULATION_FAILED, "rsx_set_option: first pass out of range");
        e->first_pass = static_cast<int>(value);
        return RSX_OK;
    case RSX_OPT_LAST_PASS:
        if (value < 0 || value > e->passes()) return fail(RSX_CALCULATION_FAILED, "rsx_set_option: last pass out of range");
        e->last_pass = static_cast<int>(value);
        return RSX_OK;
    default: return fail(RSX_INITIALIZATION_FAILED, "rsx_set_option: unknown option");
    }
}

int rsx_get_geometry(const rsx_engine* e, rsx_geometry* out)
{
    if (!e || !out) return fail(RSX_INITIALIZATION_FAILED, "rsx_get_geometry: null argument");
    out->tile_threads = kTileThreads;
    out->keys_per_thread = kKeysPerThread;
    out->tile_keys = kTileKeys;
    out->scan_block = rsx::kScanBlock;
    out->num_keys = e->n;
    out->capacity = e->capacity;
    out->num_tiles = e->ntiles(e->n);
    out->table_len = static_cast<uint64_t>(RSX_RADIX) * out->num_tiles;
    out->num_scan_blocks = static_cast<uint64_t>(RSX_RADIX) * ((out->num_tiles + rsx::kScanTiles - 1) / rsx::kScanTiles);
    out->num_passes = e->passes();
    out->key_bytes = static_cast<uint32_t>(e->key_bytes);
    out->fused_scan_resident = e->fused_scan_resident;
    out->fused_scan_max_groups = e->fused_scan_limit;
    return RSX_OK;
}

int rsx_resize(rsx_engine* e, uint64_t num_keys)
{
    if (!e) return fail(RSX_RESIZE_FAILED, "rsx_resize: null engine");
    if (num_keys > e->capacity) return fail(RSX_RESIZE_FAILED, "rsx_resize: beyond capacity");
    e->n = num_keys;
    return RSX_OK;
}

int rsx_upload(rsx_engine* e, const void* host_keys, const uint32_t* host_perm, uint64_t n)
{
    if (!e) return fail(RSX_DATA_UPLOAD_FAILED, "rsx_upload: null engine");
    if (n > e->capacity) return fail(RSX_DATA_UPLOAD_FAILED, "rsx_upload: beyond capacity");
    if (n > 0 && !host_keys) return fail(RSX_HOST_BUFFERS_FAILED, "rsx_upload: null host keys");
    if (n > 0 && e->has_payload && !host_perm) return fail(RSX_HOST_BUFFERS_FAILED, "rsx_upload: payload engine needs a permutation buffer");
    if (bind_device(e, RSX_DATA_UPLOAD_FAILED) != RSX_OK) return RSX_DATA_UPLOAD_FAILED;
    e->n = n;
    if (n > 0) {
        RSX_TRY(hipMemcpyAsync(e->keys[e->cur], host_keys, static_cast<size_t>(n) * e->key_bytes, hipMemcpyHostToDevice, e->stream),
                RSX_DATA_UPLOAD_FAILED);
        if (e->has_payload) {
            RSX_TRY(hipMemcpyAsync(e->perm[e->cur], host_perm, static_cast<size_t>(n) * 4, hipMemcpyHostToDevice, e->stream),
                    RSX_DATA_UPLOAD_FAILED);
        }
    }
    RSX_TRY(hipStreamSynchronize(e->stream), RSX_DATA_UPLOAD_FAILED);
    e->result_external = false;
    e->result_keys = e->keys[e->cur];
    e->result_perm = e->has_payload ? e->perm[e->cur] : nullptr;
    return RSX_OK;
}

int rsx_fill_pad(rsx_engine* e, uint64_t byte_offset)
{
    if (!e) return fail(RSX_CALCULATION_FAILED, "rsx_fill_pad: null engine");
    const uint64_t first = byte_offset / e->key_bytes;
    if (byte_offset % e->key_bytes != 0 || first > e->n) return fail(RSX_CALCULATION_FAILED, "rsx_fill_pad: bad offset");
    const uint64_t count = e->n - first;
    if (count == 0) return RSX_OK;
    if (bind_device(e, RSX_CALCULATION_FAILED) != RSX_OK) return RSX_CALCULATION_FAILED;
    const uint32_t blocks = static_cast<uint32_t>(std::min<uint64_t>((count + 255) / 256, 2048));
    if (e->key_bytes == 4) {
        uint32_t a = 0, m = 0;
        order_consts<uint32_t>(e, &a, &m);
        const uint32_t v = codec_decode_host<uint32_t>(0xFFFFFFFEu, a, m);
        hipLaunchKernelGGL(rsx::fill_kernel<uint32_t>, dim3(blocks), dim3(256), 0, e->stream, static_cast<uint32_t*>(e->keys[e->cur]),
                           first, count, v);
    } else {
        uint64_t a = 0, m = 0;
        order_consts<uint64_t>(e, &a, &m);
        const uint64_t v = codec_decode_host<uint64_t>(0xFFFFFFFFFFFFFFFEull, a, m);
        hipLaunchKernelGGL(rsx::fill_kernel<uint64_t>, dim3(blocks), dim3(256), 0, e->stream, static_cast<uint64_t*>(e->keys[e->cur]),
                           first, count, v);
    }
    RSX_TRY(hipGetLastError(), RSX_CALCULATION_FAILED);
    return RSX_OK;
}

int rsx_download(rsx_engine* e, void* host_keys_out, uint32_t* host_perm_out, uint32_t* hist_out, uint64_t hist_cap,
                 uint32_t* globsum_out, uint64_t globsum_cap)
{
    if (!e) return fail(RSX_DATA_DOWNLOAD_FAILED, "rsx_download: null engine");
    if (bind_device(e, RSX_DATA_DOWNLOAD_FAILED) != RSX_OK) return RSX_DATA_DOWNLOAD_FAILED;
    RSX_TRY(hipStreamSynchronize(e->stream), RSX_DATA_DOWNLOAD_FAILED);
    if (check_scan_timeout(e, RSX_DATA_DOWNLOAD_FAILED) != RSX_OK) return RSX_DATA_DOWNLOAD_FAILED;
    if (e->result_external && e->n > 0 && (host_keys_out || host_perm_out))
        return fail(RSX_DATA_DOWNLOAD_FAILED, "rsx_download: the last sort (rsx_sort_from_to) wrote into the caller's buffer; the engine holds no result");
    if (e->n > 0 && host_keys_out) {
        RSX_TRY(hipMemcpyAsync(host_keys_out, e->result_keys, static_cast<size_t>(e->n) * e->key_bytes, hipMemcpyDeviceToHost, e->stream),
                RSX_DATA_DOWNLOAD_FAILED);
    }
    if (e->n > 0 && host_perm_out && e->has_payload) {
        RSX_TRY(hipMemcpyAsync(host_perm_out, e->result_perm, static_cast<size_t>(e->n) * 4, hipMemcpyDeviceToHost, e->stream),
                RSX_DATA_DOWNLOAD_FAILED);
    }
    if (e->ref_diag && ((hist_out && hist_cap) || (globsum_out && globsum_cap))) {
        if (e->n == 0 || e->n % rsx::kRefVps != 0 || !e->last_in)
            return fail(RSX_DATA_DOWNLOAD_FAILED, "rsx_download: reference-geometry diagnostics (RSX_OPT_REF_DIAGNOSTICS) need a finished 4-BIT pass over a multiple of 1024 keys as the last pass of the sort");
// ... 607 lines not shown
```

radix-sort_amd/csrc/rsx_common.hpp:

```cpp
#pragma once

#include <hip/hip_runtime.h>
#include <stdint.h>

namespace rsx {


constexpr int kRadixBits = 4;
constexpr int kRadix = 1 << kRadixBits;
constexpr int kWave = 64;
constexpr int kNumXcd = 8;


template <typename Key>
struct alignas(16) KeyVec {
    static constexpr int N = 16 / sizeof(Key);
    Key k[N];
};

struct alignas(16) U32x4 {
    uint32_t v[4];
};

template <typename Key>
__device__ __forceinline__ KeyVec<Key> load_keys16(const Key* p)
{
    return *reinterpret_cast<const KeyVec<Key>*>(p);
}

typedef uint16_t __attribute__((may_alias)) u16_alias;
typedef uint32_t __attribute__((may_alias)) u32_alias;

template <typename Key>
__device__ __forceinline__ uint32_t digit_of(Key key, int shift, Key flip, uint32_t mask)
{
    return static_cast<uint32_t>((key ^ flip) >> shift) & mask;
}

template <typename Key>
struct KeyCodec {
    Key ea, em;
    Key da, dm;
};

__device__ __forceinline__ uint32_t sign_fill(uint32_t x) { return static_cast<uint32_t>(static_cast<int32_t>(x) >> 31); }
__device__ __forceinline__ uint64_t sign_fill(uint64_t x) { return static_cast<uint64_t>(static_cast<int64_t>(x) >> 63); }

template <typename Key>
__device__ __forceinline__ Key codec_encode(Key x, Key a, Key m)
{
    return (x ^ (sign_fill(x) & m)) ^ a;
}
template <typename Key>
__device__ __forceinline__ Key codec_decode(Key y, Key a, Key m)
{
    const Key z = y ^ a;
    return z ^ (sign_fill(z) & m);
}

__device__ __forceinline__ uint32_t ranged_bucket(uint32_t x, int shift, uint32_t mul, uint32_t mask)
{
    const uint32_t q = mul ? __umulhi(x, mul) : (x >> shift);
    return q < mask ? q : mask;
}
__device__ __forceinline__ uint32_t ranged_bucket(uint64_t x, int shift, uint64_t mul, uint32_t mask)
{
    const uint64_t q = mul ? __umul64hi(x, mul) : (x >> shift);
    return q < mask ? static_cast<uint32_t>(q) : mask;
}

constexpr int kMaxSplitters = 7;
template <typename Key>
struct SplitSet {
    Key s[kMaxSplitters];
    uint32_t n;
};

template <typename Key>
__device__ __forceinline__ uint32_t splitter_bucket(Key x, const SplitSet<Key>& set)
{
    uint32_t b = 0;
#pragma unroll
    for (int k = 0; k < kMaxSplitters; ++k) {
        if (k < static_cast<int>(set.n)) {
            b += (x > set.s[k] ? 1u : 0u) + (x >= set.s[k] ? 1u : 0u);
        }
    }
    return b;
}

__host__ __device__ __forceinline__ uint32_t tile_of_block(uint32_t bid, uint32_t tiles_per_xcd, int remap)
{
    if (!(remap & 1)) {
        return bid;
    }
    const uint32_t x = bid % kNumXcd;
    uint32_t j = bid / kNumXcd + x * (static_cast<uint32_t>(remap) >> 8);
    j = j >= tiles_per_xcd ? j - tiles_per_xcd : j;
    return x * tiles_per_xcd + j;
}

__device__ __forceinline__ uint32_t wave_inclusive_scan(uint32_t v)
{
    v += static_cast<uint32_t>(__builtin_amdgcn_update_dpp(0, static_cast<int>(v), 0x111, 0xf, 0xf, false));
    v += static_cast<uint32_t>(__builtin_amdgcn_update_dpp(0, static_cast<int>(v), 0x112, 0xf, 0xf, false));
    v += static_cast<uint32_t>(__builtin_amdgcn_update_dpp(0, static_cast<int>(v), 0x114, 0xf, 0xf, false));
    v += static_cast<uint32_t>(__builtin_amdgcn_update_dpp(0, static_cast<int>(v), 0x118, 0xf, 0xf, false));
    v += static_cast<uint32_t>(__builtin_amdgcn_update_dpp(0, static_cast<int>(v), 0x142, 0xa, 0xf, false));
    v += static_cast<uint32_t>(__builtin_amdgcn_update_dpp(0, static_cast<int>(v), 0x143, 0xc, 0xf, false));
    return v;
}

template <int THREADS, bool TRAILING_BARRIER = true>
__device__ __forceinline__ uint32_t block_exclusive_scan(uint32_t v, uint32_t* wtot, uint32_t& total)
{
    constexpr int WAVES = THREADS / kWave;
    const uint32_t lane = threadIdx.x & (kWave - 1);
    const uint32_t wave = threadIdx.x / kWave;
    const uint32_t incl = wave_inclusive_scan(v);
    if (lane == kWave - 1) {
        wtot[wave] = incl;
    }
    __syncthreads();
    uint32_t before = 0, all = 0;
#pragma unroll
    for (int w = 0; w < WAVES; ++w) {
        const uint32_t t = wtot[w];
        before += (static_cast<uint32_t>(w) < wave) ? t : 0u;
        all += t;
    }
    total = all;
    if constexpr (TRAILING_BARRIER) {
        __syncthreads();
    }
    return before + incl - v;
}

}
```

radix-sort_amd/csrc/rsx_reorder.hpp:

```cpp
#pragma once

#include "rsx_common.hpp"
#include "rsx_scan.hpp"

namespace rsx {

struct alignas(8) RunBase {
    uint32_t gbase;
    uint32_t la_base;
};

constexpr uint32_t kLaDummy = 2 * kRadix * kRadix;
constexpr int kLaReplicas = 2;

template <typename Key, bool PAYLOAD>
constexpr int la_replicas()
{
    return (PAYLOAD || sizeof(Key) != 4) ? 1 : kLaReplicas;
}
template <int REPL>
__device__ __forceinline__ void lookahead_count(uint32_t* la, uint32_t idx)
{
    const uint32_t first = static_cast<uint32_t>(__builtin_amdgcn_readfirstlane(static_cast<int>(idx)));
    if (__builtin_expect(__ballot(idx != first) == 0ull, 0)) {
        if ((threadIdx.x & (kWave - 1)) == 0) {
            atomicAdd(&la[first * REPL], static_cast<uint32_t>(kWave));
        }
    } else {
        atomicAdd(&la[idx * REPL + (threadIdx.x & (REPL - 1))], 1u);
    }
}

template <int SH>
__device__ __forceinline__ uint32_t add_lshl(uint32_t a, uint32_t b)
{
    uint32_t r;
    asm("v_add_lshl_u32 %0, %1, %2, %3" : "=v"(r) : "v"(a), "v"(b), "n"(SH));
    return r;
}

template <typename T>
__device__ __forceinline__ void lds_store_at(uint32_t byte_offset, T value)
{
    *reinterpret_cast<__attribute__((address_space(3))) T*>(static_cast<uintptr_t>(byte_offset)) = value;
}

__device__ __forceinline__ uint32_t field_word(uint32_t key, bool) { return key; }
__device__ __forceinline__ uint32_t field_word(uint64_t key, bool hi) { return hi ? static_cast<uint32_t>(key >> 32) : static_cast<uint32_t>(key); }

#ifdef RSX_STAMPS
#define RSX_STAMP(k)                                                                                      \
    do {                                                                                                  \
        if (stamp_buf && tid == 0) {                                                                      \
            unsigned long long t_;                                                                        \
            asm volatile("s_memtime %0\n\ts_waitcnt lgkmcnt(0)" : "=s"(t_)::"memory");                    \
            stamp_buf[static_cast<uint64_t>(tile) * 16 + (k)] = t_;                                       \
        }                                                                                                 \
    } while (0)
#else
#define RSX_STAMP(k) do { } while (0)
#endif

template <typename Key, int THREADS, int KPT>
struct ReorderLayout {
    static constexpr int TILE = THREADS * KPT;
    static constexpr int KD = sizeof(Key) / 4;
    static constexpr int PADSH = (KD == 1) ? 5 : 4;
    static constexpr int XELEMS = TILE + (TILE >> PADSH);
    static constexpr int XBUF_DW = XELEMS * KD;
    static constexpr int CNT_DW = 8 * THREADS;
    static constexpr int CNT_AT = XBUF_DW;
    static constexpr int IMAGE_DW = XBUF_DW + CNT_DW;
    static constexpr int WTOT_DW = 16;
    static constexpr int GBASE_DW = 2 * kRadix;
    static constexpr int LA_DW = kLaReplicas * (kRadix * 2 * kRadix + 8);
    static constexpr int SELF_DW = (THREADS / kWave) * 2 * kRadix + kRadix;
    static constexpr int TOTAL_DW = IMAGE_DW + WTOT_DW + GBASE_DW + LA_DW + SELF_DW;
    static constexpr int TILE_SHIFT = __builtin_ctz(TILE);
    static_assert((TILE & (TILE - 1)) == 0, "tile size must be a power of two (slot -> output tile by shift)");
    static_assert(THREADS % (1 << PADSH) == 0, "the padded index of slot r*THREADS+t must split into a per-thread base and a constant");
    static constexpr size_t BYTES = static_cast<size_t>(TOTAL_DW) * 4;
    static constexpr int WGS_PER_CU = static_cast<int>((160 * 1024) / BYTES);
    static constexpr int WAVES_CAP = 6;
    static constexpr int MIN_WAVES = (WGS_PER_CU * THREADS / 256) > WAVES_CAP ? WAVES_CAP : (WGS_PER_CU * THREADS / 256);
    static_assert(TILE <= 32768, "16-bit packed counters");
    static_assert(KPT % (16 / sizeof(Key)) == 0 && THREADS % 64 == 0 && THREADS % 8 == 0, "geometry");
};

template <typename Key, int THREADS, int KPT, bool PAYLOAD, bool RANGED = false>
constexpr int reorder_min_waves()
{
    constexpr int w = ReorderLayout<Key, THREADS, KPT>::MIN_WAVES;
    constexpr int cap = 4 * THREADS / 256;
    return (PAYLOAD && w > cap) ? cap : w;
}

constexpr int kSelfScanMaxTiles = 1024;
struct SelfScanArgs {
    const uint32_t* counts;
    uint32_t* zero_rows;
    uint32_t* table_out;
};

struct InlineScanArgs {
    unsigned long long* sums;
    uint32_t* scanned;
    uint32_t* temp;
    uint32_t* counts;
    uint32_t* ready;
    uint32_t* timeout;
    uint32_t epoch;
    uint32_t ngroups;
    int from_counts;
};

template <typename Key, int THREADS, int KPT, bool PAYLOAD, bool LOOKAHEAD, bool RANGED = false, bool INLINE_SCAN = false, bool CODEC = false>
__global__ __launch_bounds__(THREADS, (INLINE_SCAN ? 3 : reorder_min_waves<Key, THREADS, KPT, PAYLOAD, RANGED>())) void reorder_kernel(const Key* __restrict__ in, Key* __restrict__ out,
                                                           const uint32_t* __restrict__ pin, uint32_t* __restrict__ pout,
                                                           const uint32_t* table, uint64_t n, uint32_t ntiles,
                                                           uint32_t tiles_per_xcd, int remap, int shift, Key flip, uint32_t mask,
                                                           uint32_t* __restrict__ next_counts, int next_shift,
                                                           const uint32_t* __restrict__ globsum, Key lo, Key mul,
                                                           SplitSet<Key> split, SelfScanArgs self, InlineScanArgs iscan = InlineScanArgs{},
                                                           KeyCodec<Key> codec = KeyCodec<Key>{})
{
    static_assert(!CODEC || (!RANGED && !INLINE_SCAN), "the codec serves rsx_sort's passes and the step API only");
    static_assert(!INLINE_SCAN || (!RANGED && THREADS == kScanTiles), "the inline scan is the fused scan's workgroup: 256 threads, rsx_sort's passes only");
    using L = ReorderLayout<Key, THREADS, KPT>;
    static_assert(!(RANGED && LOOKAHEAD), "the ranged bucket function is for the one-pass partition only");
    constexpr bool RAW = LOOKAHEAD;
    constexpr int TILE = L::TILE;
    constexpr int VEC = KeyVec<Key>::N;
    constexpr int NV = KPT / VEC;
    constexpr uint32_t CNT_ROW_BYTES = THREADS * 4;

    extern __shared__ __attribute__((aligned(16))) uint32_t smem[];
    uint32_t* xbuf = smem;
    uint32_t* cnt = smem + L::CNT_AT;
    uint32_t* wtot = smem + L::IMAGE_DW;
    RunBase* runs = reinterpret_cast<RunBase*>(wtot + L::WTOT_DW);
    uint32_t* la = wtot + L::WTOT_DW + L::GBASE_DW;
    uint32_t* self_part = la + L::LA_DW;
    uint32_t* self_base = self_part + (THREADS / kWave) * 2 * kRadix;

    const uint32_t tid = threadIdx.x;
    if constexpr (INLINE_SCAN) {
        if (blockIdx.x < iscan.ngroups) {
            fused_scan_group<true, true>(*reinterpret_cast<FusedScanLds*>(smem), blockIdx.x, const_cast<uint32_t*>(table), iscan.sums, iscan.scanned, iscan.temp,
                                         ntiles, iscan.ngroups, iscan.counts, iscan.from_counts != 0, iscan.epoch, iscan.timeout, iscan.ready);
            __syncthreads();
        }
    }
    const uint32_t tile = tile_of_block(blockIdx.x, tiles_per_xcd, remap);
    if (tile >= ntiles) {
        return;
    }
    const uint64_t base = static_cast<uint64_t>(tile) * TILE;
    const uint64_t left = n - base;
    const uint32_t valid = left < static_cast<uint64_t>(TILE) ? static_cast<uint32_t>(left) : static_cast<uint32_t>(TILE);
    const bool full = (valid == TILE);
    const Key pad_key = CODEC ? codec_decode(static_cast<Key>(~Key{0}), codec.ea, codec.em) : static_cast<Key>(~flip);
#ifdef RSX_STAMPS
    unsigned long long* stamp_buf = reinterpret_cast<unsigned long long*>(const_cast<uint32_t*>(globsum));
    globsum = nullptr;
    if (stamp_buf && tid == 0) {
        unsigned long long rt_;
        asm volatile("s_memrealtime %0\n\ts_waitcnt lgkmcnt(0)" : "=s"(rt_)::"memory");
        stamp_buf[static_cast<uint64_t>(tile) * 16 + 14] = rt_;
    }
    RSX_STAMP(0);
#endif

    const bool hi_cur = sizeof(Key) == 8 && shift >= 32;
    const bool hi_next = sizeof(Key) == 8 && next_shift >= 32;
    const uint32_t sh = static_cast<uint32_t>(shift) & 31u;
    const uint32_t nsh = static_cast<uint32_t>(next_shift) & 31u;
    constexpr uint32_t flip_cur = 0u;
    const uint32_t flip_next = LOOKAHEAD ? static_cast<uint32_t>((flip >> next_shift) & Key{kRadix - 1}) : 0u;

    auto dig = [=](Key key) -> uint32_t {
        if constexpr (RANGED) {
            if (split.n) {
                return splitter_bucket(static_cast<Key>(key ^ flip), split);
            }
            return ranged_bucket(static_cast<Key>((key ^ flip) - lo), shift, mul, mask);
        } else if constexpr (RAW) {
            return __builtin_amdgcn_ubfe(field_word(key, hi_cur), sh, 4u);
        } else {
            return digit_of(key, shift, flip, mask);
        }
    };

    constexpr uint32_t RAKE_STRIDE = THREADS / 8;
    const bool rake_head = (tid % RAKE_STRIDE) == 0;
    const uint32_t hl = tid / RAKE_STRIDE;
    uint32_t first_lo = 0, first_hi = 0, group_lo = 0, group_hi = 0;
    const bool self_scan = !RANGED && self.counts != nullptr;
    if (rake_head && !self_scan && !INLINE_SCAN) {
        const uint64_t e_lo = static_cast<uint64_t>(hl) * ntiles + tile;
        const uint64_t e_hi = static_cast<uint64_t>(hl + 8) * ntiles + tile;
        first_lo = table[e_lo];
        first_hi = table[e_hi];
        if (globsum) {
            const uint32_t ngroups = (ntiles + kScanTiles - 1) / kScanTiles;
            group_lo = globsum[static_cast<uint64_t>(hl) * ngroups + tile / kScanTiles];
            group_hi = globsum[static_cast<uint64_t>(hl + 8) * ngroups + tile / kScanTiles];
        }
    }

    Key k[KPT];
    if (full) {
#pragma unroll
        for (int j = 0; j < NV; ++j) {
            const KeyVec<Key> v = load_keys16(in + base + tid * KPT + j * VEC);
#pragma unroll
            for (int e = 0; e < VEC; ++e) {
                k[j * VEC + e] = v.k[e];
            }
        }
    } else {
#pragma unroll
        for (int i = 0; i < KPT; ++i) {
            const uint32_t li = tid * KPT + i;
            k[i] = li < valid ? in[base + li] : pad_key;
        }
    }
    if constexpr (CODEC) {
#pragma unroll
        for (int i = 0; i < KPT; ++i) {
            k[i] = codec_encode(k[i], codec.ea, codec.em);
        }
    }
    uint32_t pl[PAYLOAD ? KPT : 1];
    if constexpr (PAYLOAD) {
        if (full) {
#pragma unroll
            for (int q = 0; q < KPT / 4; ++q) {
                const U32x4 x = *reinterpret_cast<const U32x4*>(pin + base + tid * KPT + q * 4);
                pl[q * 4 + 0] = x.v[0];
                pl[q * 4 + 1] = x.v[1];
                pl[q * 4 + 2] = x.v[2];
                pl[q * 4 + 3] = x.v[3];
            }
        } else {
#pragma unroll
            for (int i = 0; i < KPT; ++i) {
                const uint32_t li = tid * KPT + i;
                pl[i] = li < valid ? pin[base + li] : 0u;
            }
        }
    }

    if (self_scan) {
        const uint32_t q = tid & 3u, r = tid >> 2;
        constexpr uint32_t RS = THREADS / 4;
        const U32x4* rows = reinterpret_cast<const U32x4*>(self.counts);
        uint32_t tot[4] = {0u, 0u, 0u, 0u}, pre[4] = {0u, 0u, 0u, 0u};
        uint32_t t2 = r;
        for (; t2 + 3u * RS < ntiles; t2 += 4u * RS) {
            U32x4 v[4];
#pragma unroll
            for (int u = 0; u < 4; ++u) {
                v[u] = rows[(t2 + static_cast<uint32_t>(u) * RS) * 4u + q];
            }
#pragma unroll
            for (int u = 0; u < 4; ++u) {
                const bool earlier = t2 + static_cast<uint32_t>(u) * RS < tile;
#pragma unroll
                for (int c = 0; c < 4; ++c) {
                    tot[c] += v[u].v[c];
                    pre[c] += earlier ? v[u].v[c] : 0u;
                }
            }
        }
        for (; t2 < ntiles; t2 += RS) {
            const U32x4 v = rows[t2 * 4u + q];
#pragma unroll
            for (int c = 0; c < 4; ++c) {
                tot[c] += v.v[c];
                pre[c] += (t2 < tile) ? v.v[c] : 0u;
            }
        }
        auto same_q_sum = [](uint32_t x) -> uint32_t {
            x += static_cast<uint32_t>(__builtin_amdgcn_update_dpp(0, static_cast<int>(x), 0x124, 0xf, 0xf, false));
            x += static_cast<uint32_t>(__builtin_amdgcn_update_dpp(0, static_cast<int>(x), 0x128, 0xf, 0xf, false));
            x += __shfl_xor(x, 16);
            x += __shfl_xor(x, 32);
            return x;
        };
        const uint32_t lane = tid & (kWave - 1), wave = tid / kWave;
#pragma unroll
        for (int c = 0; c < 4; ++c) {
            tot[c] = same_q_sum(tot[c]);
            pre[c] = same_q_sum(pre[c]);
        }
        if (lane < 4u) {
#pragma unroll
            for (int c = 0; c < 4; ++c) {
                self_part[(wave * 2 + 0) * kRadix + lane * 4u + static_cast<uint32_t>(c)] = tot[c];
                self_part[(wave * 2 + 1) * kRadix + lane * 4u + static_cast<uint32_t>(c)] = pre[c];
            }
        }
        __syncthreads();
        if (tid < kRadix) {
            uint32_t total = 0, before = 0;
#pragma unroll
            for (int w = 0; w < THREADS / kWave; ++w) {
                total += self_part[(w * 2 + 0) * kRadix + tid];
                before += self_part[(w * 2 + 1) * kRadix + tid];
            }
            const uint32_t first = wave_inclusive_scan(total) - total + before;
            self_base[tid] = first;
            self.zero_rows[tile * kRadix + tid] = 0;
            if (self.table_out) {
                self.table_out[static_cast<uint64_t>(tid) * ntiles + tile] = first;
            }
        }
        __syncthreads();
        if (rake_head) {
            first_lo = self_base[hl];
            first_hi = self_base[hl + 8];
        }
    }

    static_assert(KPT <= 16, "nibble counters: a thread's count of one digit must fit 4 bits before its last key");
    u32_alias* cnt32 = reinterpret_cast<u32_alias*>(cnt);
    if constexpr (LOOKAHEAD) {
        for (uint32_t c = tid; c < static_cast<uint32_t>(L::LA_DW); c += THREADS) {
            la[c] = 0;
        }
    }
#ifdef RSX_STAMPS
    asm volatile("s_waitcnt vmcnt(0)" ::: "memory");
    RSX_STAMP(1);
#endif
    uint32_t nib[RANGED ? KPT / 8 : 1];
    auto bucket_at = [&](int i) -> uint32_t {
        if constexpr (RANGED) {
            return (nib[i >> 3] >> ((i & 7) * 4)) & 15u;
        } else {
            return dig(k[i]);
        }
    };
    if constexpr (RANGED) {
#pragma unroll
        for (int w = 0; w < KPT / 8; ++w) {
            nib[w] = 0;
        }
#pragma unroll
        for (int i = 0; i < KPT; ++i) {
            nib[i >> 3] |= dig(k[i]) << ((i & 7) * 4);
        }
    }
    uint32_t slot[KPT];
    {
        uint64_t seen = 0;
#pragma unroll
        for (int i = 0; i < KPT; ++i) {
            const uint32_t sh4 = bucket_at(i) << 2;
            slot[i] = static_cast<uint32_t>(seen >> sh4) & 15u;
            asm volatile("" : "+v"(slot[i]));
            if (i + 1 < KPT) {
                seen += 1ull << sh4;
            }
        }
        const uint32_t seen_lo = static_cast<uint32_t>(seen), seen_hi = static_cast<uint32_t>(seen >> 32);
#pragma unroll
        for (int l = 0; l < 8; ++l) {
            cnt32[l * THREADS + tid] = __builtin_amdgcn_ubfe(seen_lo, 4u * l, 4u) | (__builtin_amdgcn_ubfe(seen_hi, 4u * l, 4u) << 16);
        }
        const uint32_t d_last = bucket_at(KPT - 1);
        atomicAdd(reinterpret_cast<uint32_t*>(cnt) + (d_last & 7u) * THREADS + tid, 1u << ((d_last >> 3) * 16u));
    }
    unsigned char* cbytes = reinterpret_cast<unsigned char*>(cnt);
    auto counter_at = [&](int i) -> u16_alias* {
        if constexpr (RAW) {
            const uint32_t w = field_word(k[i], hi_cur);
            const uint32_t l3 = __builtin_amdgcn_ubfe(w, sh, 3u);
            const uint32_t h = __builtin_amdgcn_ubfe(w, sh + 3u, 1u);
            return reinterpret_cast<u16_alias*>(cbytes + (l3 * CNT_ROW_BYTES + tid * 4u) + h * 2u);
        } else {
            const uint32_t d = bucket_at(i);
            return reinterpret_cast<u16_alias*>(cbytes + ((d & 7u) * CNT_ROW_BYTES + tid * 4u) + (d >> 3) * 2u);
        }
    };
    RSX_STAMP(2);
    if constexpr (INLINE_SCAN) {
        if (tid == 0) {
            const uint32_t* word = iscan.ready + tile / kScanTiles;
            uint32_t spins = 0;
            while (__hip_atomic_load((gu32*)(word), __ATOMIC_RELAXED, __HIP_MEMORY_SCOPE_AGENT) != iscan.epoch) {
                __builtin_amdgcn_s_sleep(2);
                if (++spins > (1u << 22)) {
                    __hip_atomic_store((gu32*)(iscan.timeout), 1u, __ATOMIC_RELAXED, __HIP_MEMORY_SCOPE_SYSTEM);
                    break;
                }
            }
        }
    }
    __syncthreads();
    if constexpr (INLINE_SCAN) {
        if (rake_head) {
            first_lo = __hip_atomic_load((gu32*)(table) + static_cast<uint64_t>(hl) * ntiles + tile, __ATOMIC_RELAXED, __HIP_MEMORY_SCOPE_AGENT);
            first_hi = __hip_atomic_load((gu32*)(table) + static_cast<uint64_t>(hl + 8) * ntiles + tile, __ATOMIC_RELAXED, __HIP_MEMORY_SCOPE_AGENT);
        }
    }
    RSX_STAMP(3);

    {
        U32x4 a = *reinterpret_cast<const U32x4*>(cnt + tid * 8);
        U32x4 b = *reinterpret_cast<const U32x4*>(cnt + tid * 8 + 4);
        const uint32_t sum = a.v[0] + a.v[1] + a.v[2] + a.v[3] + b.v[0] + b.v[1] + b.v[2] + b.v[3];
        uint32_t total;
        uint32_t run = block_exclusive_scan<THREADS, false>(sum, wtot, total);
        run += total << 16;
        if (rake_head) {
            first_lo += group_lo;
            first_hi += group_hi;
            const uint32_t g_lo = first_lo - (run & 0xFFFFu), g_hi = first_hi - (run >> 16);
            const uint32_t r_lo = hl ^ flip_cur, r_hi = (hl + 8u) ^ flip_cur;
            runs[r_lo] = RunBase{g_lo, (r_lo << 5) - ((first_lo >> L::TILE_SHIFT) << 4)};
            runs[r_hi] = RunBase{g_hi, (r_hi << 5) - ((first_hi >> L::TILE_SHIFT) << 4)};
        }
        uint32_t t;
        t = a.v[0]; a.v[0] = run; run += t;
        t = a.v[1]; a.v[1] = run; run += t;
        t = a.v[2]; a.v[2] = run; run += t;
        t = a.v[3]; a.v[3] = run; run += t;
        t = b.v[0]; b.v[0] = run; run += t;
        t = b.v[1]; b.v[1] = run; run += t;
        t = b.v[2]; b.v[2] = run; run += t;
        t = b.v[3]; b.v[3] = run;
        *reinterpret_cast<U32x4*>(cnt + tid * 8) = a;
        *reinterpret_cast<U32x4*>(cnt + tid * 8 + 4) = b;
    }
    __syncthreads();
    RSX_STAMP(4);

    Key* xk = reinterpret_cast<Key*>(xbuf);
    {
        uint32_t first_of_digit[KPT];
#pragma unroll
        for (int i = 0; i < KPT; ++i) {
            first_of_digit[i] = *counter_at(i);
        }
#pragma unroll
        for (int i = 0; i < KPT; ++i) {
            slot[i] += first_of_digit[i];
        }
#pragma unroll
        for (int i = 0; i < KPT; ++i) {
            lds_store_at<Key>(add_lshl<(sizeof(Key) == 4 ? 2 : 3)>(slot[i], slot[i] >> L::PADSH), k[i]);
        }
        if constexpr (RANGED) {
            __syncthreads();
            unsigned char* staged_bucket = reinterpret_cast<unsigned char*>(cnt);
#pragma unroll
            for (int i = 0; i < KPT; ++i) {
                staged_bucket[slot[i]] = static_cast<unsigned char>(bucket_at(i));
            }
        }
    }
    __syncthreads();
    RSX_STAMP(5);

    constexpr uint32_t RSTRIDE = THREADS + (THREADS >> L::PADSH);
    const uint32_t rd_base = tid + (tid >> L::PADSH);
    Key okey[KPT];
    uint32_t g[KPT];
    uint32_t la_idx[LOOKAHEAD ? KPT : 1];
#pragma unroll
    for (int r = 0; r < KPT; ++r) {
        okey[r] = xk[rd_base + static_cast<uint32_t>(r) * RSTRIDE];
    }
    {
        RunBase rb[KPT];
#pragma unroll
        for (int r = 0; r < KPT; ++r) {
            if constexpr (RANGED) {
                rb[r] = runs[reinterpret_cast<const unsigned char*>(cnt)[static_cast<uint32_t>(r) * THREADS + tid]];
            } else {
                rb[r] = runs[dig(okey[r])];
            }
        }
#pragma unroll
        for (int r = 0; r < KPT; ++r) {
            g[r] = rb[r].gbase + tid + static_cast<uint32_t>(r) * THREADS;
            if constexpr (LOOKAHEAD) {
                la_idx[r] = rb[r].la_base + ((g[r] >> L::TILE_SHIFT) << 4) + __builtin_amdgcn_ubfe(field_word(okey[r], hi_next), nsh, 4u);
            }
        }
    }
    RSX_STAMP(6);
    if constexpr (CODEC) {
#pragma unroll
        for (int r = 0; r < KPT; ++r) {
            okey[r] = codec_decode(okey[r], codec.da, codec.dm);
        }
    }
    if (full) {
#pragma unroll
        for (int r = 0; r < KPT; ++r) {
            out[g[r]] = okey[r];
        }
    } else {
#pragma unroll
        for (int r = 0; r < KPT; ++r) {
            const uint32_t i = static_cast<uint32_t>(r) * THREADS + tid;
            if (i < valid) {
                out[g[r]] = okey[r];
            } else if constexpr (LOOKAHEAD) {
                la_idx[r] = kLaDummy;
            }
        }
    }
    RSX_STAMP(7);
    if constexpr (LOOKAHEAD) {
        const uint32_t first0 = static_cast<uint32_t>(__builtin_amdgcn_readfirstlane(static_cast<int>(la_idx[0])));
        if (__builtin_expect(__ballot(la_idx[0] != first0) != 0ull, 1)) {
            constexpr int REPL = la_replicas<Key, PAYLOAD>();
            uint32_t* la_mine = la + (tid & (REPL - 1));
#pragma unroll
            for (int r = 0; r < KPT; ++r) {
                atomicAdd(&la_mine[la_idx[r] * REPL], 1u);
            }
        } else {
#pragma unroll
            for (int r = 0; r < KPT; ++r) {
                lookahead_count<la_replicas<Key, PAYLOAD>()>(la, la_idx[r]);
            }
        }
    }
    if constexpr (PAYLOAD) {
        __syncthreads();
#pragma unroll
        for (int i = 0; i < KPT; ++i) {
            lds_store_at<uint32_t>(add_lshl<2>(slot[i], slot[i] >> 5), pl[i]);
        }
        __syncthreads();
        constexpr uint32_t PSTRIDE = THREADS + (THREADS >> 5);
        const uint32_t pd_base = tid + (tid >> 5);
        uint32_t pay[KPT];
#pragma unroll
        for (int r = 0; r < KPT; ++r) {
            pay[r] = xbuf[pd_base + static_cast<uint32_t>(r) * PSTRIDE];
        }
#pragma unroll
        for (int r = 0; r < KPT; ++r) {
            const uint32_t i = static_cast<uint32_t>(r) * THREADS + tid;
            if (full || i < valid) {
                pout[g[r]] = pay[r];
            }
        }
    }
    RSX_STAMP(8);
    if constexpr (LOOKAHEAD) {
        __syncthreads();
        RSX_STAMP(9);
        uint32_t first = tid;
        asm volatile("" : "+v"(first));
        for (uint32_t c = first; c < kLaDummy; c += THREADS) {
            constexpr int REPL = la_replicas<Key, PAYLOAD>();
            uint32_t v = la[c * REPL];
            if constexpr (REPL == 2) {
                v += la[c * REPL + 1];
            }
            if (v) {
                const uint32_t d = c >> 5, seg = (c >> 4) & 1u, d2 = (c & 15u) ^ flip_next;
                const uint32_t run_tile = ((d << 5) - runs[d].la_base) >> 4;
                atomicAdd(&next_counts[static_cast<uint64_t>(run_tile + seg) * kRadix + d2], v);
            }
        }
    }
#ifdef RSX_STAMPS
    RSX_STAMP(10);
    asm volatile("s_waitcnt vmcnt(0)" ::: "memory");
    RSX_STAMP(11);
    if (stamp_buf && tid == 0) {
        unsigned long long rt_;
        asm volatile("s_memrealtime %0\n\ts_waitcnt lgkmcnt(0)" : "=s"(rt_)::"memory");
        stamp_buf[static_cast<uint64_t>(tile) * 16 + 15] = rt_;
    }
#endif
}

}
```

Baseline: 79250 Mkeys/s.

## Add optional multi-tile grouping to look-ahead scatter and skip redundant count clears

The look-ahead scatter kernel gains a GROUP template parameter so one workgroup can process several consecutive tiles in a loop, flushing look-ahead counts once per group. This is selectable through an environment option and is off by default. The per-sort memset of the next-pass count buffer is now skipped when the buffer is known to be clean from the previous sort. This relies on the kernels leaving it zeroed, and the memset covers the full capacity when it does run.

```diff
diff --git a/radix-sort_amd/csrc/rsx_capi.hip b/radix-sort_amd/csrc/rsx_capi.hip
--- a/radix-sort_amd/csrc/rsx_capi.hip
+++ b/radix-sort_amd/csrc/rsx_capi.hip
@@ -233,6 +233,8 @@
 #endif
     long r8_extra_lds = -1;
     long reorder_extra_lds = -1;
+    int reorder_group = -1;
+    bool counts_next_dirty = true;
     int reorder_wide = -1;
     int r8_wide = -1;
     int num_cus = 0;
@@ -377,13 +379,14 @@
     int remap;
 };
 
-Grid grid_for(const rsx_engine* e, uint64_t count, uint32_t tile_keys = kTileKeys)
+Grid grid_for(const rsx_engine* e, uint64_t count, uint32_t tile_keys = kTileKeys, uint32_t group = 1)
 {
     Grid g;
     g.ntiles = static_cast<uint32_t>((count + tile_keys - 1) / tile_keys);
-    g.tiles_per_xcd = (g.ntiles + rsx::kNumXcd - 1) / rsx::kNumXcd;
-    g.blocks = e->xcd_remap ? g.tiles_per_xcd * rsx::kNumXcd : g.ntiles;
-    const uint64_t want = e->xcd_phase < 0 ? g.tiles_per_xcd / rsx::kNumXcd : static_cast<uint64_t>(e->xcd_phase);
+    const uint32_t units = (g.ntiles + group - 1) / group;
+    g.tiles_per_xcd = (units + rsx::kNumXcd - 1) / rsx::kNumXcd;
+    g.blocks = e->xcd_remap ? g.tiles_per_xcd * rsx::kNumXcd : units;
+    const uint64_t want = e->xcd_phase < 0 ? g.tiles_per_xcd / rsx::kNumXcd : static_cast<uint64_t>(e->xcd_phase) / group;
     const uint32_t phase = (e->xcd_remap && (rsx::kNumXcd - 1) * want < g.tiles_per_xcd) ? static_cast<uint32_t>(want) : 0u;
     g.remap = (e->xcd_remap ? 1 : 0) | static_cast<int>(phase << 8);
     return g;
@@ -518,18 +521,18 @@
     return RSX_OK;
 }
 
-template <typename Key, bool PAYLOAD, bool LOOKAHEAD, bool RANGED = false, int KPT = kKeysPerThread, int THREADS = kTileThreads>
+template <typename Key, bool PAYLOAD, bool LOOKAHEAD, bool RANGED = false, int KPT = kKeysPerThread, int THREADS = kTileThreads, int GROUP = 1>
 int launch_reorder_t(rsx_engine* e, const void* in, void* out, const uint32_t* pin, uint32_t* pout, uint64_t count, int shift,
                      uint32_t mask, int next_shift, Key lo = Key{0}, Key mul = Key{0}, uint32_t nsplit = 0,
                      rsx::SelfScanArgs self = rsx::SelfScanArgs{nullptr, nullptr, nullptr}, uint32_t* next_counts = nullptr, int cx = 0)
 {
     using L = rsx::ReorderLayout<Key, THREADS, KPT>;
-    const Grid g = grid_for(e, count, THREADS * KPT);
+    const Grid g = grid_for(e, count, THREADS * KPT, GROUP);
     e->last_in = in;
     e->last_shift = shift;
     Bracket b(e, PH_REORDER);
     const size_t lds = L::BYTES + (KPT != kKeysPerThread ? 0u : e->reorder_extra_lds >= 0 ? static_cast<size_t>(e->reorder_extra_lds) : (PAYLOAD && sizeof(Key) == 4 && !RANGED) ? (16u << 10) : 0u);
-    if constexpr (!RANGED) {
+    if constexpr (!RANGED && GROUP == 1) {
         if (cx) {
             hipLaunchKernelGGL((rsx::reorder_kernel<Key, THREADS, KPT, PAYLOAD, LOOKAHEAD, false, false, true>), dim3(g.blocks), dim3(THREADS), lds,
                                e->stream, static_cast<const Key*>(in), static_cast<Key*>(out), pin, pout, e->table, count,
@@ -540,7 +543,7 @@
             return RSX_OK;
         }
     }
-    hipLaunchKernelGGL((rsx::reorder_kernel<Key, THREADS, KPT, PAYLOAD, LOOKAHEAD, RANGED>), dim3(g.blocks), dim3(THREADS),
+    hipLaunchKernelGGL((rsx::reorder_kernel<Key, THREADS, KPT, PAYLOAD, LOOKAHEAD, RANGED, false, false, GROUP>), dim3(g.blocks), dim3(THREADS),
                        lds,
                        e->stream, static_cast<const Key*>(in), static_cast<Key*>(out), pin, pout, e->table, count,
                        g.ntiles, g.tiles_per_xcd, g.remap, shift, flip_mask<Key>(e), mask,
@@ -555,6 +558,23 @@
     return RSX_OK;
 }
 
+int reorder_group_for(const rsx_engine* e, bool , bool )
+{
+    return e->reorder_group > 0 ? e->reorder_group : 1;
+}
+
+template <typename Key, bool PAYLOAD, int KPT = kKeysPerThread, int THREADS = kTileThreads>
+bool launch_reorder_grouped(rsx_engine* e, int group, const void* in, void* out, const uint32_t* pin, uint32_t* pout, uint64_t count, int shift, uint32_t mask, int next_shift, int* rc)
+{
+    const rsx::SelfScanArgs none{nullptr, nullptr, nullptr};
+    switch (group) {
+    case 2: *rc = launch_reorder_t<Key, PAYLOAD, true, false, KPT, THREADS, 2>(e, in, out, pin, pout, count, shift, mask, next_shift, Key{0}, Key{0}, 0, none); return true;
+    case 4: *rc = launch_reorder_t<Key, PAYLOAD, true, false, KPT, THREADS, 4>(e, in, out, pin, pout, count, shift, mask, next_shift, Key{0}, Key{0}, 0, none); return true;
+    case 8: *rc = launch_reorder_t<Key, PAYLOAD, true, false, KPT, THREADS, 8>(e, in, out, pin, pout, count, shift, mask, next_shift, Key{0}, Key{0}, 0, none); return true;
+    default: return false;
+    }
+}
+
 template <typename Key>
 int launch_reorder(rsx_engine* e, const void* in, void* out, const uint32_t* pin, uint32_t* pout, uint64_t count, int shift,
                    uint32_t mask, int next_shift = -1, int cx = 0)
@@ -562,14 +582,21 @@
     const rsx::SelfScanArgs none{nullptr, nullptr, nullptr};
     if (count == 0) return RSX_OK;
     const bool payload = pin && pout;
+    const int group = (next_shift >= 0 && !cx && e->ntiles(count) > static_cast<uint64_t>(rsx::kSelfScanMaxTiles)) ? reorder_group_for(e, sizeof(Key) == 8, payload) : 1;
+    int grc = RSX_OK;
 #if RSX_PRODUCT_SHAPE
     if constexpr (sizeof(Key) == 8) {
         if (payload && (e->reorder_wide >= 0 ? e->reorder_wide != 0 : true)) {
+            if (group > 1 && launch_reorder_grouped<Key, true, 8, 512>(e, group, in, out, pin, pout, count, shift, mask, next_shift, &grc)) return grc;
             return next_shift >= 0 ? launch_reorder_t<Key, true, true, false, 8, 512>(e, in, out, pin, pout, count, shift, mask, next_shift, Key{0}, Key{0}, 0, none, nullptr, cx)
                                    : launch_reorder_t<Key, true, false, false, 8, 512>(e, in, out, pin, pout, count, shift, mask, 0, Key{0}, Key{0}, 0, none, nullptr, cx);
         }
     }
 #endif
+    if (group > 1 && (payload ? launch_reorder_grouped<Key, true>(e, group, in, out, pin, pout, count, shift, mask, next_shift, &grc)
+                              : launch_reorder_grouped<Key, false>(e, group, in, out, nullptr, nullptr, count, shift, mask, next_shift, &grc))) {
+        return grc;
+    }
     if (next_shift >= 0) {
         return payload ? launch_reorder_t<Key, true, true>(e, in, out, pin, pout, count, shift, mask, next_shift, Key{0}, Key{0}, 0, none, nullptr, cx)
                        : launch_reorder_t<Key, false, true>(e, in, out, nullptr, nullptr, count, shift, mask, next_shift, Key{0}, Key{0}, 0, none, nullptr, cx);
@@ -598,13 +625,27 @@
     return RSX_OK;
 }
 
-template <typename Key, bool PAYLOAD, bool LOOKAHEAD, bool RANGED = false, int KPT = kKeysPerThread, int THREADS = kTileThreads, bool CODEC = false>
+template <typename Key, bool PAYLOAD, bool LOOKAHEAD, bool RANGED = false, int KPT = kKeysPerThread, int THREADS = kTileThreads, bool CODEC = false, int GROUP = 1>
 int allow_lds()
 {
     using L = rsx::ReorderLayout<Key, THREADS, KPT>;
-    const void* fn = reinterpret_cast<const void*>(&rsx::reorder_kernel<Key, THREADS, KPT, PAYLOAD, LOOKAHEAD, RANGED, false, CODEC>);
+    const void* fn = reinterpret_cast<const void*>(&rsx::reorder_kernel<Key, THREADS, KPT, PAYLOAD, LOOKAHEAD, RANGED, false, CODEC, GROUP>);
     RSX_TRY(hipFuncSetAttribute(fn, hipFuncAttributeMaxDynamicSharedMemorySize, static_cast<int>(L::BYTES) + (64 << 10)), RSX_INITIALIZATION_FAILED);
     return no_static_lds(fn, "reorder_kernel");
+}
+
+template <int GROUP>
+int allow_lds_grouped()
+{
+    int rc = RSX_OK;
+#if RSX_PRODUCT_SHAPE
+    if (rc == RSX_OK) rc = allow_lds<uint64_t, true, true, false, 8, 512, false, GROUP>();
+#endif
+    if (rc == RSX_OK) rc = allow_lds<uint32_t, false, true, false, kKeysPerThread, kTileThreads, false, GROUP>();
+    if (rc == RSX_OK) rc = allow_lds<uint32_t, true, true, false, kKeysPerThread, kTileThreads, false, GROUP>();
+    if (rc == RSX_OK) rc = allow_lds<uint64_t, false, true, false, kKeysPerThread, kTileThreads, false, GROUP>();
+    if (rc == RSX_OK) rc = allow_lds<uint64_t, true, true, false, kKeysPerThread, kTileThreads, false, GROUP>();
+    return rc;
 }
 
 template <typename Key>
@@ -1029,14 +1070,21 @@
         return sort_selfscan_enqueue<Key>(e, ext_keys, ext_perm, count);
     }
 #if defined(RSX_EXPERIMENTS) && RSX_PRODUCT_SHAPE
-    if (!e->codec() && inline_scan_takes(e, count)) return sort_inline_enqueue<Key>(e, ext_keys, ext_perm, count);
+    if (!e->codec() && inline_scan_takes(e, count)) {
+        e->counts_next_dirty = true;
+        return sort_inline_enqueue<Key>(e, ext_keys, ext_perm, count);
+    }
 #endif
     const void* in = ext_keys ? ext_keys : e->keys[e->cur];
     const uint32_t* pin = e->has_payload ? (ext_keys ? ext_perm : e->perm[e->cur]) : nullptr;
     int dst = ext_keys ? e->cur : (e->cur ^ 1);
     Bracket whole(e, PH_TOTAL);
     if (e->lookahead && count > 0) {
-        RSX_TRY(hipMemsetAsync(e->counts_next, 0, static_cast<size_t>(e->ntiles(count)) * RSX_RADIX * 4, e->stream), RSX_CALCULATION_FAILED);
+        if (e->counts_next_dirty || e->use_graph) {
+            const size_t all = ((e->ntiles(e->capacity) + rsx::kScanTiles - 1) / rsx::kScanTiles) * rsx::kScanTiles * RSX_RADIX * 4;
+            RSX_TRY(hipMemsetAsync(e->counts_next, 0, all, e->stream), RSX_CALCULATION_FAILED);
+        }
+        e->counts_next_dirty = true;
     }
     for (int pass = e->first_pass; pass < e->last_pass; ++pass) {
         const bool to_caller = e->final_keys_out && pass + 1 == e->last_pass;
@@ -1065,6 +1113,7 @@
         pin = pout;
         dst ^= 1;
     }
+    if (e->lookahead && count > 0) e->counts_next_dirty = false;
     if (in == e->keys[0] || in == e->keys[1]) {
         e->cur = (in == e->keys[0]) ? 0 : 1;
     }
@@ -1169,6 +1218,7 @@
     volatile uint32_t* flag = e->scan_timeout_host;
     if (*flag != 0) {
         *flag = 0;
+        e->counts_next_dirty = true;
         return fail(status, "the fused table scan timed out waiting for a group sum: the result of that sort is undefined (reported once; the engine remains usable)");
     }
     return RSX_OK;
@@ -1249,6 +1299,8 @@
     {"RSX_RADIX_BITS", "8: byte-wide passes in the sort chain (RSX_OPT_RADIX_BITS)", [](rsx_engine* e, const char* v) { e->radix_bits = std::atoi(v) == 8 ? 8 : 4; }},
     {"RSX_RADIX8_MIN_KEYS", "8-bit passes only above this many keys (default 2^19)", [](rsx_engine* e, const char* v) { e->radix8_min_keys = std::max<uint64_t>(std::strtoull(v, nullptr, 10), kTileKeys); }},
     {"RSX_REORDER_EXTRA_LDS_KB", "unused dynamic LDS per 4-bit scatter workgroup = fewer per CU (-1: per-variant policy)", [](rsx_engine* e, const char* v) { e->reorder_extra_lds = kb_or_policy(v, 64); }},
+    {"RSX_REORDER_TILE_GROUP", "consecutive tiles per workgroup of the look-ahead scatter, counts flushed once per group (1, 2, 4, 8; -1: policy)",
+     [](rsx_engine* e, const char* v) { const int g = std::atoi(v); e->reorder_group = (g == 1 || g == 2 || g == 4 || g == 8) ? g : -1; }},
     {"RSX_REORDER_WIDE", "4-bit scatter of 64-bit keys + payload on 512 x 8 (0 / 1, -1: policy = on)", [](rsx_engine* e, const char* v) { e->reorder_wide = std::max(-1, std::min(1, std::atoi(v))); }},
     {"RSX_R8_EXTRA_LDS_KB", "the same for the 8-bit scatter (-1: per-variant policy)", [](rsx_engine* e, const char* v) { e->r8_extra_lds = kb_or_policy(v, 96); }},
     {"RSX_R8_PACKED", "0: uint32 key and payload travel apart through the 8-bit scatter (default 1: one 64-bit element)", [](rsx_engine* e, const char* v) { e->r8_packed = std::atoi(v) != 0; }},
@@ -1456,6 +1508,9 @@
     if (rc == RSX_OK) rc = allow_lds<uint32_t, true, true>();
     if (rc == RSX_OK) rc = allow_lds<uint64_t, false, true>();
     if (rc == RSX_OK) rc = allow_lds<uint64_t, true, true>();
+    if (rc == RSX_OK) rc = allow_lds_grouped<2>();
+    if (rc == RSX_OK) rc = allow_lds_grouped<4>();
+    if (rc == RSX_OK) rc = allow_lds_grouped<8>();
     if (rc == RSX_OK) rc = allow_lds<uint32_t, false, false, true>();
     if (rc == RSX_OK) rc = allow_lds<uint32_t, true, false, true>();
     if (rc == RSX_OK) rc = allow_lds<uint64_t, false, false, true>();
diff --git a/radix-sort_amd/csrc/rsx_common.hpp b/radix-sort_amd/csrc/rsx_common.hpp
--- a/radix-sort_amd/csrc/rsx_common.hpp
+++ b/radix-sort_amd/csrc/rsx_common.hpp
@@ -112,11 +112,11 @@
 }
 
 template <int THREADS, bool TRAILING_BARRIER = true>
-__device__ __forceinline__ uint32_t block_exclusive_scan(uint32_t v, uint32_t* wtot, uint32_t& total)
+__device__ __forceinline__ uint32_t block_exclusive_scan(uint32_t v, uint32_t* wtot, uint32_t& total, uint32_t tid = threadIdx.x)
 {
     constexpr int WAVES = THREADS / kWave;
-    const uint32_t lane = threadIdx.x & (kWave - 1);
-    const uint32_t wave = threadIdx.x / kWave;
+    const uint32_t lane = tid & (kWave - 1);
+    const uint32_t wave = tid / kWave;
     const uint32_t incl = wave_inclusive_scan(v);
     if (lane == kWave - 1) {
         wtot[wave] = incl;
diff --git a/radix-sort_amd/csrc/rsx_reorder.hpp b/radix-sort_amd/csrc/rsx_reorder.hpp
--- a/radix-sort_amd/csrc/rsx_reorder.hpp
+++ b/radix-sort_amd/csrc/rsx_reorder.hpp
@@ -114,7 +114,7 @@
     int from_counts;
 };
 
-template <typename Key, int THREADS, int KPT, bool PAYLOAD, bool LOOKAHEAD, bool RANGED = false, bool INLINE_SCAN = false, bool CODEC = false>
+template <typename Key, int THREADS, int KPT, bool PAYLOAD, bool LOOKAHEAD, bool RANGED = false, bool INLINE_SCAN = false, bool CODEC = false, int GROUP = 1>
 __global__ __launch_bounds__(THREADS, (INLINE_SCAN ? 3 : reorder_min_waves<Key, THREADS, KPT, PAYLOAD, RANGED>())) void reorder_kernel(const Key* __restrict__ in, Key* __restrict__ out,
                                                            const uint32_t* __restrict__ pin, uint32_t* __restrict__ pout,
                                                            const uint32_t* table, uint64_t n, uint32_t ntiles,
@@ -128,6 +128,7 @@
     static_assert(!INLINE_SCAN || (!RANGED && THREADS == kScanTiles), "the inline scan is the fused scan's workgroup: 256 threads, rsx_sort's passes only");
     using L = ReorderLayout<Key, THREADS, KPT>;
     static_assert(!(RANGED && LOOKAHEAD), "the ranged bucket function is for the one-pass partition only");
+    static_assert(GROUP == 1 || (LOOKAHEAD && !INLINE_SCAN && !CODEC && GROUP <= 16), "tile groups serve the look-ahead passes of the large-table chain");
     constexpr bool RAW = LOOKAHEAD;
     constexpr int TILE = L::TILE;
     constexpr int VEC = KeyVec<Key>::N;
@@ -142,8 +143,9 @@
     uint32_t* la = wtot + L::WTOT_DW + L::GBASE_DW;
     uint32_t* self_part = la + L::LA_DW;
     uint32_t* self_base = self_part + (THREADS / kWave) * 2 * kRadix;
-
-    const uint32_t tid = threadIdx.x;
+    uint32_t* run_first = self_part;
+
+    uint32_t tid = threadIdx.x;
     if constexpr (INLINE_SCAN) {
         if (blockIdx.x < iscan.ngroups) {
             fused_scan_group<true, true>(*reinterpret_cast<FusedScanLds*>(smem), blockIdx.x, const_cast<uint32_t*>(table), iscan.sums, iscan.scanned, iscan.temp,
@@ -151,409 +153,472 @@
             __syncthreads();
         }
     }
-    const uint32_t tile = tile_of_block(blockIdx.x, tiles_per_xcd, remap);
-    if (tile >= ntiles) {
+    const uint32_t first_tile = tile_of_block(blockIdx.x, tiles_per_xcd, remap) * GROUP;
+    if (first_tile >= ntiles) {
         return;
     }
-    const uint64_t base = static_cast<uint64_t>(tile) * TILE;
-    const uint64_t left = n - base;
-    const uint32_t valid = left < static_cast<uint64_t>(TILE) ? static_cast<uint32_t>(left) : static_cast<uint32_t>(TILE);
-    const bool full = (valid == TILE);
-    const Key pad_key = CODEC ? codec_decode(static_cast<Key>(~Key{0}), codec.ea, codec.em) : static_cast<Key>(~flip);
-#ifdef RSX_STAMPS
-    unsigned long long* stamp_buf = reinterpret_cast<unsigned long long*>(const_cast<uint32_t*>(globsum));
-    globsum = nullptr;
-    if (stamp_buf && tid == 0) {
-        unsigned long long rt_;
-        asm volatile("s_memrealtime %0\n\ts_waitcnt lgkmcnt(0)" : "=s"(rt_)::"memory");
-        stamp_buf[static_cast<uint64_t>(tile) * 16 + 14] = rt_;
-    }
-    RSX_STAMP(0);
-#endif
-
     const bool hi_cur = sizeof(Key) == 8 && shift >= 32;
     const bool hi_next = sizeof(Key) == 8 && next_shift >= 32;
     const uint32_t sh = static_cast<uint32_t>(shift) & 31u;
     const uint32_t nsh = static_cast<uint32_t>(next_shift) & 31u;
     constexpr uint32_t flip_cur = 0u;
     const uint32_t flip_next = LOOKAHEAD ? static_cast<uint32_t>((flip >> next_shift) & Key{kRadix - 1}) : 0u;
-
-    auto dig = [=](Key key) -> uint32_t {
+#ifdef RSX_STAMPS
+    unsigned long long* stamp_buf = reinterpret_cast<unsigned long long*>(const_cast<uint32_t*>(globsum));
+    globsum = nullptr;
+#endif
+    uint32_t gi = 0;
+#pragma unroll 1
+    do {
+        const uint32_t tile = first_tile + gi;
+        if (GROUP > 1 && tile >= ntiles) {
+            break;
+        }
+        if constexpr (GROUP > 1) {
+            asm volatile("" : "+v"(tid));
+        }
+        const uint64_t base = static_cast<uint64_t>(tile) * TILE;
+        const uint64_t left = n - base;
+        const uint32_t valid = left < static_cast<uint64_t>(TILE) ? static_cast<uint32_t>(left) : static_cast<uint32_t>(TILE);
+        const bool full = (valid == TILE);
+        const Key pad_key = CODEC ? codec_decode(static_cast<Key>(~Key{0}), codec.ea, codec.em) : static_cast<Key>(~flip);
+#ifdef RSX_STAMPS
+        if (stamp_buf && tid == 0) {
+            unsigned long long rt_;
+            asm volatile("s_memrealtime %0\n\ts_waitcnt lgkmcnt(0)" : "=s"(rt_)::"memory");
+            stamp_buf[static_cast<uint64_t>(tile) * 16 + 14] = rt_;
+        }
+        RSX_STAMP(0);
+#endif
+
+        auto dig = [=](Key key) -> uint32_t {
+            if constexpr (RANGED) {
+                if (split.n) {
+                    return splitter_bucket(static_cast<Key>(key ^ flip), split);
+                }
+                return ranged_bucket(static_cast<Key>((key ^ flip) - lo), shift, mul, mask);
+            } else if constexpr (RAW) {
+                return __builtin_amdgcn_ubfe(field_word(key, hi_cur), sh, 4u);
+            } else {
+                return digit_of(key, shift, flip, mask);
+            }
+        };
+
+        constexpr uint32_t RAKE_STRIDE = THREADS / 8;
+        const bool rake_head = (tid % RAKE_STRIDE) == 0;
+        const uint32_t hl = tid / RAKE_STRIDE;
+        uint32_t first_lo = 0, first_hi = 0, group_lo = 0, group_hi = 0;
+        const bool self_scan = !RANGED && GROUP == 1 && self.counts != nullptr;
+        if (rake_head && !self_scan && !INLINE_SCAN) {
+            const uint64_t e_lo = static_cast<uint64_t>(hl) * ntiles + tile;
+            const uint64_t e_hi = static_cast<uint64_t>(hl + 8) * ntiles + tile;
+            first_lo = table[e_lo];
+            first_hi = table[e_hi];
+            if (globsum) {
+                const uint32_t ngroups = (ntiles + kScanTiles - 1) / kScanTiles;
+                group_lo = globsum[static_cast<uint64_t>(hl) * ngroups + tile / kScanTiles];
+                group_hi = globsum[static_cast<uint64_t>(hl + 8) * ngroups + tile / kScanTiles];
+            }
+        }
+
+        Key k[KPT];
+        if (full) {
+#pragma unroll
+            for (int j = 0; j < NV; ++j) {
+                const KeyVec<Key> v = load_keys16(in + base + tid * KPT + j * VEC);
+#pragma unroll
+                for (int e = 0; e < VEC; ++e) {
+                    k[j * VEC + e] = v.k[e];
+                }
+            }
+        } else {
+#pragma unroll
+            for (int i = 0; i < KPT; ++i) {
+                const uint32_t li = tid * KPT + i;
+                k[i] = li < valid ? in[base + li] : pad_key;
+            }
+        }
+        if constexpr (CODEC) {
+#pragma unroll
+            for (int i = 0; i < KPT; ++i) {
+                k[i] = codec_encode(k[i], codec.ea, codec.em);
+            }
+        }
+        uint32_t pl[PAYLOAD ? KPT : 1];
+        if constexpr (PAYLOAD) {
+            if (full) {
+#pragma unroll
+                for (int q = 0; q < KPT / 4; ++q) {
+                    const U32x4 x = *reinterpret_cast<const U32x4*>(pin + base + tid * KPT + q * 4);
+                    pl[q * 4 + 0] = x.v[0];
+                    pl[q * 4 + 1] = x.v[1];
+                    pl[q * 4 + 2] = x.v[2];
+                    pl[q * 4 + 3] = x.v[3];
+                }
+            } else {
+#pragma unroll
+                for (int i = 0; i < KPT; ++i) {
+                    const uint32_t li = tid * KPT + i;
+                    pl[i] = li < valid ? pin[base + li] : 0u;
+                }
+            }
+        }
+
+        if (self_scan) {
+            const uint32_t q = tid & 3u, r = tid >> 2;
+            constexpr uint32_t RS = THREADS / 4;
+            const U32x4* rows = reinterpret_cast<const U32x4*>(self.counts);
+            uint32_t tot[4] = {0u, 0u, 0u, 0u}, pre[4] = {0u, 0u, 0u, 0u};
+            uint32_t t2 = r;
+            for (; t2 + 3u * RS < ntiles; t2 += 4u * RS) {
+                U32x4 v[4];
+#pragma unroll
+                for (int u = 0; u < 4; ++u) {
+                    v[u] = rows[(t2 + static_cast<uint32_t>(u) * RS) * 4u + q];
+                }
+#pragma unroll
+                for (int u = 0; u < 4; ++u) {
+                    const bool earlier = t2 + static_cast<uint32_t>(u) * RS < tile;
+#pragma unroll
+                    for (int c = 0; c < 4; ++c) {
+                        tot[c] += v[u].v[c];
+                        pre[c] += earlier ? v[u].v[c] : 0u;
+                    }
+                }
+            }
+            for (; t2 < ntiles; t2 += RS) {
+                const U32x4 v = rows[t2 * 4u + q];
+#pragma unroll
+                for (int c = 0; c < 4; ++c) {
+                    tot[c] += v.v[c];
+                    pre[c] += (t2 < tile) ? v.v[c] : 0u;
+                }
+            }
+            auto same_q_sum = [](uint32_t x) -> uint32_t {
+                x += static_cast<uint32_t>(__builtin_amdgcn_update_dpp(0, static_cast<int>(x), 0x124, 0xf, 0xf, false));
+                x += static_cast<uint32_t>(__builtin_amdgcn_update_dpp(0, static_cast<int>(x), 0x128, 0xf, 0xf, false));
+                x += __shfl_xor(x, 16);
+                x += __shfl_xor(x, 32);
+                return x;
+            };
+            const uint32_t lane = tid & (kWave - 1), wave = tid / kWave;
+#pragma unroll
+            for (int c = 0; c < 4; ++c) {
+                tot[c] = same_q_sum(tot[c]);
+                pre[c] = same_q_sum(pre[c]);
+            }
+            if (lane < 4u) {
+#pragma unroll
+                for (int c = 0; c < 4; ++c) {
+                    self_part[(wave * 2 + 0) * kRadix + lane * 4u + static_cast<uint32_t>(c)] = tot[c];
+                    self_part[(wave * 2 + 1) * kRadix + lane * 4u + static_cast<uint32_t>(c)] = pre[c];
+                }
+            }
+            __syncthreads();
+            if (tid < kRadix) {
+                uint32_t total = 0, before = 0;
+#pragma unroll
+                for (int w = 0; w < THREADS / kWave; ++w) {
+                    total += self_part[(w * 2 + 0) * kRadix + tid];
+                    before += self_part[(w * 2 + 1) * kRadix + tid];
+                }
+                const uint32_t first = wave_inclusive_scan(total) - total + before;
+                self_base[tid] = first;
+                self.zero_rows[tile * kRadix + tid] = 0;
+                if (self.table_out) {
+                    self.table_out[static_cast<uint64_t>(tid) * ntiles + tile] = first;
+                }
+            }
+            __syncthreads();
+            if (rake_head) {
+                first_lo = self_base[hl];
+                first_hi = self_base[hl + 8];
+            }
+        }
+
+        static_assert(KPT <= 16, "nibble counters: a thread's count of one digit must fit 4 bits before its last key");
+        u32_alias* cnt32 = reinterpret_cast<u32_alias*>(cnt);
+        if constexpr (LOOKAHEAD) {
+            if (GROUP == 1 || gi == 0) {
+                for (uint32_t c = tid; c < static_cast<uint32_t>(L::LA_DW); c += THREADS) {
+                    la[c] = 0;
+                }
+            }
+        }
+#ifdef RSX_STAMPS
+        asm volatile("s_waitcnt vmcnt(0)" ::: "memory");
+        RSX_STAMP(1);
+#endif
+        uint32_t nib[RANGED ? KPT / 8 : 1];
+        auto bucket_at = [&](int i) -> uint32_t {
+            if constexpr (RANGED) {
+                return (nib[i >> 3] >> ((i & 7) * 4)) & 15u;
+            } else {
+                return dig(k[i]);
+            }
+        };
         if constexpr (RANGED) {
-            if (split.n) {
-                return splitter_bucket(static_cast<Key>(key ^ flip), split);
-            }
-            return ranged_bucket(static_cast<Key>((key ^ flip) - lo), shift, mul, mask);
-        } else if constexpr (RAW) {
-            return __builtin_amdgcn_ubfe(field_word(key, hi_cur), sh, 4u);
+#pragma unroll
+            for (int w = 0; w < KPT / 8; ++w) {
+                nib[w] = 0;
+            }
+#pragma unroll
+            for (int i = 0; i < KPT; ++i) {
+                nib[i >> 3] |= dig(k[i]) << ((i & 7) * 4);
+            }
+        }
+        uint32_t slot[KPT];
+        {
+            uint64_t seen = 0;
+#pragma unroll
+            for (int i = 0; i < KPT; ++i) {
+                const uint32_t sh4 = bucket_at(i) << 2;
+                slot[i] = static_cast<uint32_t>(seen >> sh4) & 15u;
+                asm volatile("" : "+v"(slot[i]));
+                if (i + 1 < KPT) {
+                    seen += 1ull << sh4;
+                }
+            }
+            const uint32_t seen_lo = static_cast<uint32_t>(seen), seen_hi = static_cast<uint32_t>(seen >> 32);
+#pragma unroll
+            for (int l = 0; l < 8; ++l) {
+                cnt32[l * THREADS + tid] = __builtin_amdgcn_ubfe(seen_lo, 4u * l, 4u) | (__builtin_amdgcn_ubfe(seen_hi, 4u * l, 4u) << 16);
+            }
+            const uint32_t d_last = bucket_at(KPT - 1);
+            atomicAdd(reinterpret_cast<uint32_t*>(cnt) + (d_last & 7u) * THREADS + tid, 1u << ((d_last >> 3) * 16u));
+        }
+        unsigned char* cbytes = reinterpret_cast<unsigned char*>(cnt);
+        auto counter_at = [&](int i) -> u16_alias* {
+            if constexpr (RAW) {
+                const uint32_t w = field_word(k[i], hi_cur);
+                const uint32_t l3 = __builtin_amdgcn_ubfe(w, sh, 3u);
+                const uint32_t h = __builtin_amdgcn_ubfe(w, sh + 3u, 1u);
+                return reinterpret_cast<u16_alias*>(cbytes + (l3 * CNT_ROW_BYTES + tid * 4u) + h * 2u);
+            } else {
+                const uint32_t d = bucket_at(i);
+                return reinterpret_cast<u16_alias*>(cbytes + ((d & 7u) * CNT_ROW_BYTES + tid * 4u) + (d >> 3) * 2u);
+            }
+        };
+        RSX_STAMP(2);
+        if constexpr (INLINE_SCAN) {
+            if (tid == 0) {
+                const uint32_t* word = iscan.ready + tile / kScanTiles;
+                uint32_t spins = 0;
+                while (__hip_atomic_load((gu32*)(word), __ATOMIC_RELAXED, __HIP_MEMORY_SCOPE_AGENT) != iscan.epoch) {
+                    __builtin_amdgcn_s_sleep(2);
+                    if (++spins > (1u << 22)) {
+                        __hip_atomic_store((gu32*)(iscan.timeout), 1u, __ATOMIC_RELAXED, __HIP_MEMORY_SCOPE_SYSTEM);
+                        break;
+                    }
+                }
+            }
+        }
+        __syncthreads();
+        if constexpr (INLINE_SCAN) {
+            if (rake_head) {
+                first_lo = __hip_atomic_load((gu32*)(table) + static_cast<uint64_t>(hl) * ntiles + tile, __ATOMIC_RELAXED, __HIP_MEMORY_SCOPE_AGENT);
+                first_hi = __hip_atomic_load((gu32*)(table) + static_cast<uint64_t>(hl + 8) * ntiles + tile, __ATOMIC_RELAXED, __HIP_MEMORY_SCOPE_AGENT);
+            }
+        }
+        RSX_STAMP(3);
+
+        {
+            U32x4 a = *reinterpret_cast<const U32x4*>(cnt + tid * 8);
+            U32x4 b = *reinterpret_cast<const U32x4*>(cnt + tid * 8 + 4);
+            const uint32_t sum = a.v[0] + a.v[1] + a.v[2] + a.v[3] + b.v[0] + b.v[1] + b.v[2] + b.v[3];
+            uint32_t total;
+            uint32_t run = block_exclusive_scan<THREADS, false>(sum, wtot, total, tid);
+            run += total << 16;
+            if (rake_head) {
+                first_lo += group_lo;
+                first_hi += group_hi;
+                const uint32_t g_lo = first_lo - (run & 0xFFFFu), g_hi = first_hi - (run >> 16);
+                const uint32_t r_lo = hl ^ flip_cur, r_hi = (hl + 8u) ^ flip_cur;
+                if constexpr (GROUP > 1) {
+                    runs[r_lo].gbase = g_lo;
+                    runs[r_hi].gbase = g_hi;
+                    run_first[r_lo] = first_lo;
+                    run_first[r_hi] = first_hi;
+                } else {
+                    runs[r_lo] = RunBase{g_lo, (r_lo << 5) - ((first_lo >> L::TILE_SHIFT) << 4)};
+                    runs[r_hi] = RunBase{g_hi, (r_hi << 5) - ((first_hi >> L::TILE_SHIFT) << 4)};
+                }
+            }
+            uint32_t t;
+            t = a.v[0]; a.v[0] = run; run += t;
+            t = a.v[1]; a.v[1] = run; run += t;
+            t = a.v[2]; a.v[2] = run; run += t;
+            t = a.v[3]; a.v[3] = run; run += t;
+            t = b.v[0]; b.v[0] = run; run += t;
+            t = b.v[1]; b.v[1] = run; run += t;
+            t = b.v[2]; b.v[2] = run; run += t;
+            t = b.v[3]; b.v[3] = run;
+            *reinterpret_cast<U32x4*>(cnt + tid * 8) = a;
+            *reinterpret_cast<U32x4*>(cnt + tid * 8 + 4) = b;
+        }
+        __syncthreads();
+        RSX_STAMP(4);
+        if constexpr (GROUP > 1) {
+            if (tid < kWave) {
+                const uint32_t d = tid & (kRadix - 1);
+                const uint32_t first = run_first[d];
+                const uint32_t local = first - runs[d].gbase;
+                const uint32_t d1 = (d + 1u) & (kRadix - 1);
+                const uint32_t local_next = d == kRadix - 1 ? valid : run_first[d1] - runs[d1].gbase;
+                const uint32_t count = local_next - local;
+                const uint32_t base_tile = ((d << 5) - runs[d].la_base) >> 4;
+                bool flush = gi != 0 && tid < kRadix && count != 0 && ((first + count - 1u) >> L::TILE_SHIFT) > base_tile + 1u;
+#ifdef RSX_NO_EARLY_FLUSH
+                flush = false;
+#endif
+                uint64_t need = __ballot(flush);
+                if (__builtin_expect(need != 0ull, 0)) {
+                    constexpr int REPL = la_replicas<Key, PAYLOAD>();
+                    while (need) {
+                        const uint32_t fd = static_cast<uint32_t>(__builtin_ctzll(need));
+                        need &= need - 1;
+                        const uint32_t bt = static_cast<uint32_t>(__builtin_amdgcn_readlane(static_cast<int>(base_tile), static_cast<int>(fd)));
+                        if (tid < 2 * kRadix) {
+                            const uint32_t c = (fd << 5) + tid;
+                            uint32_t v = la[c * REPL];
+                            la[c * REPL] = 0;
+                            if constexpr (REPL == 2) {
+                                v += la[c * REPL + 1];
+                                la[c * REPL + 1] = 0;
+                            }
+                            if (v) {
+                                atomicAdd(&next_counts[static_cast<uint64_t>(bt + (tid >> 4)) * kRadix + ((tid & 15u) ^ flip_next)], v);
+                            }
+                        }
+                    }
+                }
+                if (tid < kRadix && (gi == 0 || flush)) {
+                    runs[d].la_base = (d << 5) - ((first >> L::TILE_SHIFT) << 4);
+                }
+            }
+        }
+
+        Key* xk = reinterpret_cast<Key*>(xbuf);
+        {
+            uint32_t first_of_digit[KPT];
+#pragma unroll
+            for (int i = 0; i < KPT; ++i) {
+                first_of_digit[i] = *counter_at(i);
+            }
+#pragma unroll
+            for (int i = 0; i < KPT; ++i) {
+                slot[i] += first_of_digit[i];
+            }
+#pragma unroll
+            for (int i = 0; i < KPT; ++i) {
+                lds_store_at<Key>(add_lshl<(sizeof(Key) == 4 ? 2 : 3)>(slot[i], slot[i] >> L::PADSH), k[i]);
+            }
+            if constexpr (RANGED) {
+                __syncthreads();
+                unsigned char* staged_bucket = reinterpret_cast<unsigned char*>(cnt);
+#pragma unroll
+                for (int i = 0; i < KPT; ++i) {
+                    staged_bucket[slot[i]] = static_cast<unsigned char>(bucket_at(i));
+                }
+            }
+        }
+        __syncthreads();
+        RSX_STAMP(5);
+
+        constexpr uint32_t RSTRIDE = THREADS + (THREADS >> L::PADSH);
+        const uint32_t rd_base = tid + (tid >> L::PADSH);
+        Key okey[KPT];
+        uint32_t g[KPT];
+        uint32_t la_idx[LOOKAHEAD ? KPT : 1];
+#pragma unroll
+        for (int r = 0; r < KPT; ++r) {
+            okey[r] = xk[rd_base + static_cast<uint32_t>(r) * RSTRIDE];
+        }
+        {
+            RunBase rb[KPT];
+#pragma unroll
+            for (int r = 0; r < KPT; ++r) {
+                if constexpr (RANGED) {
+                    rb[r] = runs[reinterpret_cast<const unsigned char*>(cnt)[static_cast<uint32_t>(r) * THREADS + tid]];
+                } else {
+                    rb[r] = runs[dig(okey[r])];
+                }
+            }
+#pragma unroll
+            for (int r = 0; r < KPT; ++r) {
+                g[r] = rb[r].gbase + tid + static_cast<uint32_t>(r) * THREADS;
+                if constexpr (LOOKAHEAD) {
+                    la_idx[r] = rb[r].la_base + ((g[r] >> L::TILE_SHIFT) << 4) + __builtin_amdgcn_ubfe(field_word(okey[r], hi_next), nsh, 4u);
+                }
+            }
+        }
+        RSX_STAMP(6);
+        if constexpr (CODEC) {
+#pragma unroll
+            for (int r = 0; r < KPT; ++r) {
+                okey[r] = codec_decode(okey[r], codec.da, codec.dm);
+            }
+        }
+        if (full) {
+#pragma unroll
+            for (int r = 0; r < KPT; ++r) {
+                out[g[r]] = okey[r];
+            }
         } else {
-            return digit_of(key, shift, flip, mask);
-        }
-    };
-
-    constexpr uint32_t RAKE_STRIDE = THREADS / 8;
-    const bool rake_head = (tid % RAKE_STRIDE) == 0;
-    const uint32_t hl = tid / RAKE_STRIDE;
-    uint32_t first_lo = 0, first_hi = 0, group_lo = 0, group_hi = 0;
-    const bool self_scan = !RANGED && self.counts != nullptr;
-    if (rake_head && !self_scan && !INLINE_SCAN) {
-        const uint64_t e_lo = static_cast<uint64_t>(hl) * ntiles + tile;
-        const uint64_t e_hi = static_cast<uint64_t>(hl + 8) * ntiles + tile;
-        first_lo = table[e_lo];
-        first_hi = table[e_hi];
-        if (globsum) {
-            const uint32_t ngroups = (ntiles + kScanTiles - 1) / kScanTiles;
-            group_lo = globsum[static_cast<uint64_t>(hl) * ngroups + tile / kScanTiles];
-            group_hi = globsum[static_cast<uint64_t>(hl + 8) * ngroups + tile / kScanTiles];
-        }
-    }
-
-    Key k[KPT];
-    if (full) {
-#pragma unroll
-        for (int j = 0; j < NV; ++j) {
-            const KeyVec<Key> v = load_keys16(in + base + tid * KPT + j * VEC);
-#pragma unroll
-            for (int e = 0; e < VEC; ++e) {
-                k[j * VEC + e] = v.k[e];
-            }
-        }
-    } else {
-#pragma unroll
-        for (int i = 0; i < KPT; ++i) {
-            const uint32_t li = tid * KPT + i;
-            k[i] = li < valid ? in[base + li] : pad_key;
-        }
-    }
-    if constexpr (CODEC) {
-#pragma unroll
-        for (int i = 0; i < KPT; ++i) {
-            k[i] = codec_encode(k[i], codec.ea, codec.em);
-        }
-    }
-    uint32_t pl[PAYLOAD ? KPT : 1];
-    if constexpr (PAYLOAD) {
-        if (full) {
-#pragma unroll
-            for (int q = 0; q < KPT / 4; ++q) {
-                const U32x4 x = *reinterpret_cast<const U32x4*>(pin + base + tid * KPT + q * 4);
-                pl[q * 4 + 0] = x.v[0];
-                pl[q * 4 + 1] = x.v[1];
-                pl[q * 4 + 2] = x.v[2];
-                pl[q * 4 + 3] = x.v[3];
-            }
-        } else {
-#pragma unroll
-            for (int i = 0; i < KPT; ++i) {
-                const uint32_t li = tid * KPT + i;
-                pl[i] = li < valid ? pin[base + li] : 0u;
-            }
-        }
-    }
-
-    if (self_scan) {
-        const uint32_t q = tid & 3u, r = tid >> 2;
-        constexpr uint32_t RS = THREADS / 4;
-        const U32x4* rows = reinterpret_cast<const U32x4*>(self.counts);
-        uint32_t tot[4] = {0u, 0u, 0u, 0u}, pre[4] = {0u, 0u, 0u, 0u};
-        uint32_t t2 = r;
-        for (; t2 + 3u * RS < ntiles; t2 += 4u * RS) {
-            U32x4 v[4];
-#pragma unroll
-            for (int u = 0; u < 4; ++u) {
-                v[u] = rows[(t2 + static_cast<uint32_t>(u) * RS) * 4u + q];
-            }
-#pragma unroll
-            for (int u = 0; u < 4; ++u) {
-                const bool earlier = t2 + static_cast<uint32_t>(u) * RS < tile;
-#pragma unroll
-                for (int c = 0; c < 4; ++c) {
-                    tot[c] += v[u].v[c];
-                    pre[c] += earlier ? v[u].v[c] : 0u;
-                }
-            }
-        }
-        for (; t2 < ntiles; t2 += RS) {
-            const U32x4 v = rows[t2 * 4u + q];
-#pragma unroll
-            for (int c = 0; c < 4; ++c) {
-                tot[c] += v.v[c];
-                pre[c] += (t2 < tile) ? v.v[c] : 0u;
-            }
-        }
-        auto same_q_sum = [](uint32_t x) -> uint32_t {
-            x += static_cast<uint32_t>(__builtin_amdgcn_update_dpp(0, static_cast<int>(x), 0x124, 0xf, 0xf, false));
-            x += static_cast<uint32_t>(__builtin_amdgcn_update_dpp(0, static_cast<int>(x), 0x128, 0xf, 0xf, false));
-            x += __shfl_xor(x, 16);
-            x += __shfl_xor(x, 32);
-            return x;
-        };
-        const uint32_t lane = tid & (kWave - 1), wave = tid / kWave;
-#pragma unroll
-        for (int c = 0; c < 4; ++c) {
-            tot[c] = same_q_sum(tot[c]);
-            pre[c] = same_q_sum(pre[c]);
-        }
-        if (lane < 4u) {
-#pragma unroll
-            for (int c = 0; c < 4; ++c) {
-                self_part[(wave * 2 + 0) * kRadix + lane * 4u + static_cast<uint32_t>(c)] = tot[c];
-                self_part[(wave * 2 + 1) * kRadix + lane * 4u + static_cast<uint32_t>(c)] = pre[c];
-            }
-        }
-        __syncthreads();
-        if (tid < kRadix) {
-            uint32_t total = 0, before = 0;
-#pragma unroll
-            for (int w = 0; w < THREADS / kWave; ++w) {
-                total += self_part[(w * 2 + 0) * kRadix + tid];
-                before += self_part[(w * 2 + 1) * kRadix + tid];
-            }
-            const uint32_t first = wave_inclusive_scan(total) - total + before;
-            self_base[tid] = first;
-            self.zero_rows[tile * kRadix + tid] = 0;
-            if (self.table_out) {
-                self.table_out[static_cast<uint64_t>(tid) * ntiles + tile] = first;
-            }
-        }
-        __syncthreads();
-        if (rake_head) {
-            first_lo = self_base[hl];
-            first_hi = self_base[hl + 8];
-        }
-    }
-
-    static_assert(KPT <= 16, "nibble counters: a thread's count of one digit must fit 4 bits before its last key");
-    u32_alias* cnt32 = reinterpret_cast<u32_alias*>(cnt);
-    if constexpr (LOOKAHEAD) {
-        for (uint32_t c = tid; c < static_cast<uint32_t>(L::LA_DW); c += THREADS) {
-            la[c] = 0;
-        }
-    }
+#pragma unroll
+            for (int r = 0; r < KPT; ++r) {
+                const uint32_t i = static_cast<uint32_t>(r) * THREADS + tid;
+                if (i < valid) {
+                    out[g[r]] = okey[r];
+                } else if constexpr (LOOKAHEAD) {
+                    la_idx[r] = kLaDummy;
+                }
+            }
+        }
+        RSX_STAMP(7);
+        if constexpr (LOOKAHEAD) {
+            const uint32_t first0 = static_cast<uint32_t>(__builtin_amdgcn_readfirstlane(static_cast<int>(la_idx[0])));
+            if (__builtin_expect(__ballot(la_idx[0] != first0) != 0ull, 1)) {
+                constexpr int REPL = la_replicas<Key, PAYLOAD>();
+                uint32_t* la_mine = la + (tid & (REPL - 1));
+#pragma unroll
+                for (int r = 0; r < KPT; ++r) {
+                    atomicAdd(&la_mine[la_idx[r] * REPL], 1u);
+                }
+            } else {
+#pragma unroll
+                for (int r = 0; r < KPT; ++r) {
+                    lookahead_count<la_replicas<Key, PAYLOAD>()>(la, la_idx[r]);
+                }
+            }
+        }
+        if constexpr (PAYLOAD) {
+            __syncthreads();
+#pragma unroll
+            for (int i = 0; i < KPT; ++i) {
+                lds_store_at<uint32_t>(add_lshl<2>(slot[i], slot[i] >> 5), pl[i]);
+            }
+            __syncthreads();
+            constexpr uint32_t PSTRIDE = THREADS + (THREADS >> 5);
+            const uint32_t pd_base = tid + (tid >> 5);
+            uint32_t pay[KPT];
+#pragma unroll
+            for (int r = 0; r < KPT; ++r) {
+                pay[r] = xbuf[pd_base + static_cast<uint32_t>(r) * PSTRIDE];
+            }
+#pragma unroll
+            for (int r = 0; r < KPT; ++r) {
+                const uint32_t i = static_cast<uint32_t>(r) * THREADS + tid;
+                if (full || i < valid) {
+                    pout[g[r]] = pay[r];
+                }
+            }
+        }
+        RSX_STAMP(8);
+    } while (GROUP > 1 && ++gi < static_cast<uint32_t>(GROUP));
 #ifdef RSX_STAMPS
-    asm volatile("s_waitcnt vmcnt(0)" ::: "memory");
-    RSX_STAMP(1);
+    const uint32_t tile = first_tile;
 #endif
-    uint32_t nib[RANGED ? KPT / 8 : 1];
-    auto bucket_at = [&](int i) -> uint32_t {
-        if constexpr (RANGED) {
-            return (nib[i >> 3] >> ((i & 7) * 4)) & 15u;
-        } else {
-            return dig(k[i]);
-        }
-    };
-    if constexpr (RANGED) {
-#pragma unroll
-        for (int w = 0; w < KPT / 8; ++w) {
-            nib[w] = 0;
-        }
-#pragma unroll
-        for (int i = 0; i < KPT; ++i) {
-            nib[i >> 3] |= dig(k[i]) << ((i & 7) * 4);
-        }
-    }
-    uint32_t slot[KPT];
-    {
-        uint64_t seen = 0;
-#pragma unroll
-        for (int i = 0; i < KPT; ++i) {
-            const uint32_t sh4 = bucket_at(i) << 2;
-            slot[i] = static_cast<uint32_t>(seen >> sh4) & 15u;
-            asm volatile("" : "+v"(slot[i]));
-            if (i + 1 < KPT) {
-                seen += 1ull << sh4;
-            }
-        }
-        const uint32_t seen_lo = static_cast<uint32_t>(seen), seen_hi = static_cast<uint32_t>(seen >> 32);
-#pragma unroll
-        for (int l = 0; l < 8; ++l) {
-            cnt32[l * THREADS + tid] = __builtin_amdgcn_ubfe(seen_lo, 4u * l, 4u) | (__builtin_amdgcn_ubfe(seen_hi, 4u * l, 4u) << 16);
-        }
-        const uint32_t d_last = bucket_at(KPT - 1);
-        atomicAdd(reinterpret_cast<uint32_t*>(cnt) + (d_last & 7u) * THREADS + tid, 1u << ((d_last >> 3) * 16u));
-    }
-    unsigned char* cbytes = reinterpret_cast<unsigned char*>(cnt);
-    auto counter_at = [&](int i) -> u16_alias* {
-        if constexpr (RAW) {
-            const uint32_t w = field_word(k[i], hi_cur);
-            const uint32_t l3 = __builtin_amdgcn_ubfe(w, sh, 3u);
-            const uint32_t h = __builtin_amdgcn_ubfe(w, sh + 3u, 1u);
-            return reinterpret_cast<u16_alias*>(cbytes + (l3 * CNT_ROW_BYTES + tid * 4u) + h * 2u);
-        } else {
-            const uint32_t d = bucket_at(i);
-            return reinterpret_cast<u16_alias*>(cbytes + ((d & 7u) * CNT_ROW_BYTES + tid * 4u) + (d >> 3) * 2u);
-        }
-    };
-    RSX_STAMP(2);
-    if constexpr (INLINE_SCAN) {
-        if (tid == 0) {
-            const uint32_t* word = iscan.ready + tile / kScanTiles;
-            uint32_t spins = 0;
-            while (__hip_atomic_load((gu32*)(word), __ATOMIC_RELAXED, __HIP_MEMORY_SCOPE_AGENT) != iscan.epoch) {
-                __builtin_amdgcn_s_sleep(2);
-                if (++spins > (1u << 22)) {
-                    __hip_atomic_store((gu32*)(iscan.timeout), 1u, __ATOMIC_RELAXED, __HIP_MEMORY_SCOPE_SYSTEM);
-                    break;
-                }
-            }
-        }
-    }
-    __syncthreads();
-    if constexpr (INLINE_SCAN) {
-        if (rake_head) {
-            first_lo = __hip_atomic_load((gu32*)(table) + static_cast<uint64_t>(hl) * ntiles + tile, __ATOMIC_RELAXED, __HIP_MEMORY_SCOPE_AGENT);
-            first_hi = __hip_atomic_load((gu32*)(table) + static_cast<uint64_t>(hl + 8) * ntiles + tile, __ATOMIC_RELAXED, __HIP_MEMORY_SCOPE_AGENT);
-        }
-    }
-    RSX_STAMP(3);
-
-    {
-        U32x4 a = *reinterpret_cast<const U32x4*>(cnt + tid * 8);
-        U32x4 b = *reinterpret_cast<const U32x4*>(cnt + tid * 8 + 4);
-        const uint32_t sum = a.v[0] + a.v[1] + a.v[2] + a.v[3] + b.v[0] + b.v[1] + b.v[2] + b.v[3];
-        uint32_t total;
-        uint32_t run = block_exclusive_scan<THREADS, false>(sum, wtot, total);
-        run += total << 16;
-        if (rake_head) {
-            first_lo += group_lo;
-            first_hi += group_hi;
-            const uint32_t g_lo = first_lo - (run & 0xFFFFu), g_hi = first_hi - (run >> 16);
-            const uint32_t r_lo = hl ^ flip_cur, r_hi = (hl + 8u) ^ flip_cur;
-            runs[r_lo] = RunBase{g_lo, (r_lo << 5) - ((first_lo >> L::TILE_SHIFT) << 4)};
-            runs[r_hi] = RunBase{g_hi, (r_hi << 5) - ((first_hi >> L::TILE_SHIFT) << 4)};
-        }
-        uint32_t t;
-        t = a.v[0]; a.v[0] = run; run += t;
-        t = a.v[1]; a.v[1] = run; run += t;
-        t = a.v[2]; a.v[2] = run; run += t;
-        t = a.v[3]; a.v[3] = run; run += t;
-        t = b.v[0]; b.v[0] = run; run += t;
-        t = b.v[1]; b.v[1] = run; run += t;
-        t = b.v[2]; b.v[2] = run; run += t;
-        t = b.v[3]; b.v[3] = run;
-        *reinterpret_cast<U32x4*>(cnt + tid * 8) = a;
-        *reinterpret_cast<U32x4*>(cnt + tid * 8 + 4) = b;
-    }
-    __syncthreads();
-    RSX_STAMP(4);
-
-    Key* xk = reinterpret_cast<Key*>(xbuf);
-    {
-        uint32_t first_of_digit[KPT];
-#pragma unroll
-        for (int i = 0; i < KPT; ++i) {
-            first_of_digit[i] = *counter_at(i);
-        }
-#pragma unroll
-        for (int i = 0; i < KPT; ++i) {
-            slot[i] += first_of_digit[i];
-        }
-#pragma unroll
-        for (int i = 0; i < KPT; ++i) {
-            lds_store_at<Key>(add_lshl<(sizeof(Key) == 4 ? 2 : 3)>(slot[i], slot[i] >> L::PADSH), k[i]);
-        }
-        if constexpr (RANGED) {
-            __syncthreads();
-            unsigned char* staged_bucket = reinterpret_cast<unsigned char*>(cnt);
-#pragma unroll
-            for (int i = 0; i < KPT; ++i) {
-                staged_bucket[slot[i]] = static_cast<unsigned char>(bucket_at(i));
-            }
-        }
-    }
-    __syncthreads();
-    RSX_STAMP(5);
-
-    constexpr uint32_t RSTRIDE = THREADS + (THREADS >> L::PADSH);
-    const uint32_t rd_base = tid + (tid >> L::PADSH);
-    Key okey[KPT];
-    uint32_t g[KPT];
-    uint32_t la_idx[LOOKAHEAD ? KPT : 1];
-#pragma unroll
-    for (int r = 0; r < KPT; ++r) {
-        okey[r] = xk[rd_base + static_cast<uint32_t>(r) * RSTRIDE];
-    }
-    {
-        RunBase rb[KPT];
-#pragma unroll
-        for (int r = 0; r < KPT; ++r) {
-            if constexpr (RANGED) {
-                rb[r] = runs[reinterpret_cast<const unsigned char*>(cnt)[static_cast<uint32_t>(r) * THREADS + tid]];
-            } else {
-                rb[r] = runs[dig(okey[r])];
-            }
-        }
-#pragma unroll
-        for (int r = 0; r < KPT; ++r) {
-            g[r] = rb[r].gbase + tid + static_cast<uint32_t>(r) * THREADS;
-            if constexpr (LOOKAHEAD) {
-                la_idx[r] = rb[r].la_base + ((g[r] >> L::TILE_SHIFT) << 4) + __builtin_amdgcn_ubfe(field_word(okey[r], hi_next), nsh, 4u);
-            }
-        }
-    }
-    RSX_STAMP(6);
-    if constexpr (CODEC) {
-#pragma unroll
-        for (int r = 0; r < KPT; ++r) {
-            okey[r] = codec_decode(okey[r], codec.da, codec.dm);
-        }
-    }
-    if (full) {
-#pragma unroll
-        for (int r = 0; r < KPT; ++r) {
-            out[g[r]] = okey[r];
-        }
-    } else {
-#pragma unroll
-        for (int r = 0; r < KPT; ++r) {
-            const uint32_t i = static_cast<uint32_t>(r) * THREADS + tid;
-            if (i < valid) {
-                out[g[r]] = okey[r];
-            } else if constexpr (LOOKAHEAD) {
-                la_idx[r] = kLaDummy;
-            }
-        }
-    }
-    RSX_STAMP(7);
-    if constexpr (LOOKAHEAD) {
-        const uint32_t first0 = static_cast<uint32_t>(__builtin_amdgcn_readfirstlane(static_cast<int>(la_idx[0])));
-        if (__builtin_expect(__ballot(la_idx[0] != first0) != 0ull, 1)) {
-            constexpr int REPL = la_replicas<Key, PAYLOAD>();
-            uint32_t* la_mine = la + (tid & (REPL - 1));
-#pragma unroll
-            for (int r = 0; r < KPT; ++r) {
-                atomicAdd(&la_mine[la_idx[r] * REPL], 1u);
-            }
-        } else {
-#pragma unroll
-            for (int r = 0; r < KPT; ++r) {
-                lookahead_count<la_replicas<Key, PAYLOAD>()>(la, la_idx[r]);
-            }
-        }
-    }
-    if constexpr (PAYLOAD) {
-        __syncthreads();
-#pragma unroll
-        for (int i = 0; i < KPT; ++i) {
-            lds_store_at<uint32_t>(add_lshl<2>(slot[i], slot[i] >> 5), pl[i]);
-        }
-        __syncthreads();
-        constexpr uint32_t PSTRIDE = THREADS + (THREADS >> 5);
-        const uint32_t pd_base = tid + (tid >> 5);
-        uint32_t pay[KPT];
-#pragma unroll
-        for (int r = 0; r < KPT; ++r) {
-            pay[r] = xbuf[pd_base + static_cast<uint32_t>(r) * PSTRIDE];
-        }
-#pragma unroll
-        for (int r = 0; r < KPT; ++r) {
-            const uint32_t i = static_cast<uint32_t>(r) * THREADS + tid;
-            if (full || i < valid) {
-                pout[g[r]] = pay[r];
-            }
-        }
-    }
-    RSX_STAMP(8);
     if constexpr (LOOKAHEAD) {
         __syncthreads();
         RSX_STAMP(9);
```

Result: no change. 79130 Mkeys/s (-0.1%).
